# andreicuceu/vega

Measured on AMD Instinct MI355X. Metric: model+chi2 evals/sec (Lya auto+cross), higher is better.
Workload: dtype f64

## Files before the change

vega_amd/csrc/vegamx.hip:

```cpp
#include "vmx_device.h"
#include "vmx_fit.h"
#include "vmx_ensemble.h"
#include "vmx_nested.h"
#include "vmx_smc.h"
#include "vmx_chain.h"

#include <atomic>
#include <cmath>
#include <chrono>
#include <thread>
#include <algorithm>
#include <cstdio>
#include <cstdlib>
#include <cstring>
#include <map>
#include <mutex>
#include <queue>
#include <utility>
#include <string>
#include <vector>

#ifndef VMX_MAX_LANES
#define VMX_MAX_LANES 2
#endif
// ... 11 lines not shown
            return fail(-2, std::string(#call) + ": " + hipGetErrorString(err__));           \
    } while (0)

#define REQUIRE(cond, msg)                                                                   \
    do { if (!(cond)) return fail(-1, std::string("invalid argument: ") + msg); } while (0)

namespace {

static const uint64_t VMX_PART_SENTINEL = 0x7ff8dead0000beefull;


enum KernelClass {
    KC_PROLOGUE = 0, KC_PK, KC_FFTLOG, KC_XI, KC_METAL, KC_ASSEMBLE, KC_DISTORTION, KC_POST,
    KC_INVCOV, KC_CHI2, KC_MATVEC, KC_OTHER, KC_QUAD
};
const char* kKernelNames[VMX_N_KERNELS] = {
    "prologue", "pk_multipoles", "fftlog_spline_product", "xi_bins", "metal_matrix_product",
    "assemble", "distortion_product", "post", "invcov_product", "chi2", "matvec_api", "other",
    "quadratic_form_product"};

template <typename T>
struct DevBuf {
    T* p = nullptr;
    size_t n = 0;
    bool borrowed = false;
    DevBuf() = default;
    DevBuf(const DevBuf& o) : p(o.p), n(o.n), borrowed(true) {}
    DevBuf& operator=(const DevBuf& o) { if (this != &o) { release(); p = o.p; n = o.n; borrowed = true; } return *this; }
    void forget() { if (borrowed) { p = nullptr; n = 0; borrowed = false; } }
    int alloc(size_t count, bool zero = true) {
        release();
        if (count == 0) count = 1;
        hipError_t err = hipMalloc((void**)&p, count * sizeof(T));
        if (err != hipSuccess) return fail(-2, std::string("hipMalloc: ") + hipGetErrorString(err));
        n = count;
        if (zero) {
            err = hipMemset(p, 0, count * sizeof(T));
            if (err != hipSuccess) return fail(-2, std::string("hipMemset: ") + hipGetErrorString(err));
        }
        return 0;
    }
    int upload(const T* host, size_t count) {
        if (alloc(count, false)) return -2;
        hipError_t err = hipMemcpy(p, host, count * sizeof(T), hipMemcpyHostToDevice);
        if (err != hipSuccess) return fail(-2, std::string("hipMemcpy: ") + hipGetErrorString(err));
        return 0;
    }
    void release() { if (p && !borrowed) (void)hipFree(p); p = nullptr; n = 0; borrowed = false; }
    ~DevBuf() { release(); }
};

static int upload_padded(DevBuf<double>& buf, const double* host, int rows, int cols, int ld)
{
    if (buf.alloc((size_t)rows * ld, true)) return -2;
    hipError_t err = hipMemcpy2D(buf.p, (size_t)ld * sizeof(double), host, (size_t)cols * sizeof(double),
                                 (size_t)cols * sizeof(double), rows, hipMemcpyHostToDevice);
    if (err != hipSuccess) return fail(-2, std::string("hipMemcpy2D: ") + hipGetErrorString(err));
    return 0;
}

static std::vector<double> half_form(const double* c, int n)
{
    std::vector<double> out((size_t)n * n, 0.0);
    for (int i = 0; i < n; ++i) {
        for (int j = 0; j < i; ++j) out[(size_t)i * n + j] = 0.5 * (c[(size_t)i * n + j] + c[(size_t)j * n + i]);
        out[(size_t)i * n + i] = 0.5 * c[(size_t)i * n + i];
    }
    return out;
}

struct MetalHost {
    MetalDev dev{};
    DevBuf<double> mat, svec, basis, kron_a, kron_b;
    int rows = 0, cols = 0;
};

struct ItemHost {
    ItemDev dev{};
    std::vector<MetalHost*> metals;
    DevBuf<double> dm, cinv, data, vec, dist, res, z, mock_pool, add_vec;
    DevBuf<double> marg, marg_out;
    DevBuf<double> q_mat, q_w, q_lin, q_c0, q_x0, q_x, q_z;
    DevBuf<double> q_u, q_f, q_u0, q_y;
    DevBuf<double> mg_g, mg_c0, mg_y;
    DevBuf<double> mc_chol, mc_fid, q_cfull, q_m0, mc_z, mc_noise, mc_r0, mc_t;
    bool has_factor = false;
    std::vector<double> h_q_c0;
    DevBuf<int64_t> q_basis_off;
    int q_rows = 0;
    int n_templates = 0;
    int n_mocks = 0;
    DevBuf<int32_t> inv_mask;
    DevBuf<int64_t> csr_ptr; DevBuf<int32_t> csr_idx; DevBuf<double> csr_val;
    int64_t csr_nnz = 0; bool has_csr = false;
    std::vector<int32_t> mask_idx;
    bool has_dm = false, has_cinv = false, has_mask = false, has_data = false;
    bool lean_pair = false;
};

struct FitWorkspace {
    DevBuf<double> state;
    DevBuf<vmx_migrad::Spec> spec;
    DevBuf<double> base, theta, chi2;
    DevBuf<int32_t> mock_row, count, offset, done, mock, status;
    DevBuf<double> ox[vmx_migrad::MAX_STAGES], oext[vmx_migrad::MAX_STAGES], oV[vmx_migrad::MAX_STAGES], ofval[vmx_migrad::MAX_STAGES], oedm[vmx_migrad::MAX_STAGES];
    DevBuf<int32_t> oflags[vmx_migrad::MAX_STAGES], oiter[vmx_migrad::MAX_STAGES];
    DevBuf<int64_t> onfcn[vmx_migrad::MAX_STAGES];
    int32_t* pin_word = nullptr; int32_t* dpin_word = nullptr;
    std::vector<hipEvent_t> ev_gap;
    ~FitWorkspace() {
        if (pin_word) (void)hipHostFree(pin_word);
        for (auto& ev : ev_gap) (void)hipEventDestroy(ev);
    }
};
template <typename T>
static int ensure(DevBuf<T>& b, size_t count) { return b.n >= count && b.p ? 0 : b.alloc(count, false); }

struct BoxDev {
    double* theta; const double* chi2; const int32_t* status;
    const double* fixed; const int32_t* inv; const double* lo; const double* hi;
};
struct BoxWorkspace {
    DevBuf<double> theta, chi2, fixed, lo, hi;
    DevBuf<int32_t> status, inv;
    int upload(size_t rows, int P, int n, const double* h_fixed, const double* h_lo, const double* h_hi, const std::vector<int32_t>& h_inv,
               hipStream_t st, BoxDev& D)
    {
        if (ensure(theta, rows * P) || ensure(chi2, rows) || ensure(status, rows) || ensure(fixed, P) || ensure(inv, P) || ensure(lo, n) ||
            ensure(hi, n)) return -2;
        HIP_OK(hipMemcpyAsync(fixed.p, h_fixed, (size_t)P * sizeof(double), hipMemcpyHostToDevice, st));
        HIP_OK(hipMemcpyAsync(inv.p, h_inv.data(), (size_t)P * sizeof(int32_t), hipMemcpyHostToDevice, st));
        HIP_OK(hipMemcpyAsync(lo.p, h_lo, (size_t)n * sizeof(double), hipMemcpyHostToDevice, st));
        HIP_OK(hipMemcpyAsync(hi.p, h_hi, (size_t)n * sizeof(double), hipMemcpyHostToDevice, st));
        D = BoxDev{theta.p, chi2.p, status.p, fixed.p, inv.p, lo.p, hi.p};
        return 0;
    }
};

template <int THREADS, typename U>
__device__ inline void write_cube_rows(const BoxDev& B, int P, size_t row0, int rows, U u)
{
    for (int p = threadIdx.x % 64; p < P; p += 64) {
        const int d = B.inv[p];
        const double fixed = B.fixed[p], lo = d < 0 ? 0.0 : B.lo[d], hi = d < 0 ? 0.0 : B.hi[d];
#pragma unroll 4
        for (int r = threadIdx.x / 64; r < rows; r += THREADS / 64) {
            double v = fixed;
            if (d >= 0) v = vmx_ns::map_cube(lo, hi, u(r, d));
            B.theta[(row0 + (size_t)r) * P + p] = v;
        }
    }
}
template <int THREADS, typename U>
__device__ inline void write_cube_rows(const BoxDev& B, int P, int rows, U u)
{
    write_cube_rows<THREADS>(B, P, (size_t)0, rows, u);
}

struct EnsWorkspace {
    BoxWorkspace box;
    DevBuf<double> x, lnl, prop, factor, chain, chain_lnl;
    DevBuf<int64_t> acc, n_box, n_fail;
    DevBuf<int32_t> inside, col;
    DevBuf<int32_t> mock;
    DevBuf<uint64_t> streams;
    DevBuf<double> beta;
// ... 1349 lines not shown
}

struct SmcSetDev {
    SmcDev run0;
    const int32_t* active;
    const uint64_t* streams;
    const int64_t* stage0;
    const int32_t* mock_row;
    int32_t* mock;
    int32_t rec_rows;
};

__device__ __forceinline__ SmcDev smc_view(const SmcSetDev& S, int& run)
{
    SmcDev D = S.run0;
    const size_t a = blockIdx.x, r = (size_t)S.active[a], N = (size_t)D.N, n = (size_t)D.n;
    run = (int)r;
    D.u += r * N * n; D.lnl += r * N; D.u2 += r * N * n; D.lnl2 += r * N; D.w += r * N; D.cum += r * N;
    D.mean += r * n; D.cov += r * n * n; D.chol += r * n * n; D.state += r * 2;
    D.prop += r * N * n; D.uacc += r * N; D.inside += r * N;
    D.box.theta += a * N * (size_t)D.P; D.box.chi2 += a * N; D.box.status += a * N;
    D.rec += r * (size_t)S.rec_rows * VMX_SMC_REC; D.rec_lnl += r * (size_t)S.rec_rows * N; D.rec_anc += r * (size_t)S.rec_rows * N;
    D.counters += r * 3; D.host += r * 4;
    D.stream = S.streams[r];
    return D;
}

__device__ __forceinline__ void smc_write_mock(const SmcSetDev& S, int run)
{
    if (!S.mock_row) return;
    const int N = S.run0.N, m = S.mock_row[run];
    for (int i = threadIdx.x; i < N; i += SMC_THREADS) S.mock[(size_t)blockIdx.x * N + i] = m;
}

__global__ __launch_bounds__(SMC_THREADS) void k_smc_start(SmcSetDev S)
{
    int run;
    const SmcDev D = smc_view(S, run);
    smc_write_mock(S, run);
    smc_start(D);
}

__global__ __launch_bounds__(SMC_THREADS) void k_smc_start_lnl(SmcSetDev S)
{
    int run;
    const SmcDev D = smc_view(S, run);
    smc_start_lnl(D);
}

__global__ __launch_bounds__(SMC_THREADS) void k_smc_stage(SmcSetDev S, int64_t round)
{
    int run;
    const SmcDev D = smc_view(S, run);
    smc_stage(D, S.stage0[run] + round, round);
}

__global__ __launch_bounds__(SMC_THREADS) void k_smc_stage_kept(SmcSetDev S, int64_t round, double* rec_u)
{
    int run;
    const SmcDev D = smc_view(S, run);
    if (rec_u) rec_u += (size_t)run * (size_t)S.rec_rows * (size_t)D.N * (size_t)D.n;
    smc_stage<true>(D, S.stage0[run] + round, round, rec_u);
}

__global__ __launch_bounds__(SMC_THREADS) void k_smc_move(SmcSetDev S, int64_t round, int s_dec, int s_prop)
{
    int run;
    const SmcDev D = smc_view(S, run);
    if (s_dec < 0) smc_write_mock(S, run);
    smc_move(D, S.stage0[run] + round, s_dec, s_prop, round);
}

}

struct vmx_chain_store {
    vmx_engine* engine = nullptr;
    int E = 0, W = 0, n = 0;
    int64_t capacity = 0, rows = 0;
    DevBuf<double> x, lnl;
    DevBuf<double> sums, centred, out;
    DevBuf<int64_t> window;
};

struct vmx_engine {
    int device = 0;
    hipStream_t stream = nullptr;
    hipStream_t cur = nullptr;
    std::vector<hipStream_t> aux;
    hipEvent_t ev_fork = nullptr;
    std::vector<hipEvent_t> ev_join;
    bool finalized = false;
    std::vector<vmx_engine*> lanes;
    int n_lanes = 1;
    int64_t lane_calls = 0;
    hipStream_t last_stream = nullptr;
    const int32_t* call_mock = nullptr;
    FitWorkspace* fitws = nullptr;
    EnsWorkspace* ensws = nullptr;
    std::vector<vmx_chain_store*> chain_stores;
    vmx_chain_store* chain_store = nullptr;
    NsWorkspace* nsws = nullptr;
    SmcWorkspace* smcws = nullptr;
    hipEvent_t lane_wait = nullptr, ev_rows = nullptr, ev_lane = nullptr;

    int nk = 0, nkp = 0, n_mu = 0;
    int n_rows = 0, n_extra = 0, mu_lo = 0, mu_hi = 0;
    int mu_tiers = 1;
    vmx_plan::MuTierDesc mu_tier[vmx_plan::MU_TIERS] = {};
    std::vector<uint16_t> zmap64, zmap16;
    int last_tab2_kt = 0;
    DevBuf<double> node_w, mu_img, mu_img_w;
    std::vector<int32_t> rule_slot; std::vector<double> rule_lo, rule_hi;
    DevBuf<int32_t> d_rule_slot; DevBuf<double> d_rule_lo, d_rule_hi;
    double k_node_max = 0.0; bool mu_nodes_on = true;
    DevBuf<double> k, pklin, delta2, mu, sq1mmu2, lnmu, wl, gk, gk_mom, fv_x, fv_f, xtab;
    std::vector<int32_t> const_slots;
    std::vector<int32_t> const_slots2;
    DevBuf<int32_t> d_const_slots, d_const_slots2, d_xtab_pipe, d_xtab_partner;
    DevBuf<double> xtab_k;
    std::vector<int32_t> xi_static_taps, xi_static_bins;
    DevBuf<int32_t> d_xi_static_taps, d_xi_static_bins;
    DevBuf<unsigned long long> gemm_trace;
    size_t gemm_trace_blocks = 0;
    DevBuf<unsigned long long> pk_trace;
    size_t pk_trace_blocks = 0;
    std::vector<int32_t> w_groups;
    DevBuf<int32_t> d_w_groups;
    bool no_pk_w = false;
    std::vector<Tab2Group> tab2_groups;
    DevBuf<double> xtab_key;
    int n_xtab = 0;
    int const_hint = 0;
    int fv_n = 0;
    struct GkSpec { double rp, rt, mock_rp, mock_rt; };
    std::vector<GkSpec> gk_tables;
    std::vector<double> h_k, h_mu;

    int n_coef = 0, ncp = 0, n_knots = 0;
    DevBuf<double> op;
    bool op_set[VMX_MAX_ELL] = {false, false, false, false};
    bool extrapolate = false;
    double x0[VMX_MAX_ELL] = {0}, h[VMX_MAX_ELL] = {0};

    std::vector<PipeDev> pipes;
    std::vector<double> h_r, h_mu_c, h_z, h_relz, h_lnrelz, h_lnrelz2, h_growth;
    DevBuf<double> cr, cmu, crp, crt, cz, crelz, clnrelz, clnrelz2, cgrowth;
    DevBuf<PipeDev> d_pipes;
    std::vector<PkGroup> pk_groups;
    DevBuf<PkGroup> d_pk_groups;
    std::vector<int32_t> pk_members, pk_poly, pk_static;
    DevBuf<int32_t> d_pk_members, d_pk_poly, d_pk_static, d_pipe_active;
    DevBuf<double> poly_coef, poly_bins;
    int64_t poly_bins_total = 0;
    int n_active = 0;
    bool poly_dirty = true;

    std::vector<ItemHost*> items;
    std::vector<MetalHost*> metals;
    DevBuf<ItemDev> d_items;
    DevBuf<MetalDev> d_metals;
    std::vector<double> h_bb, h_odd, h_odd_op;
    std::map<int, int64_t> odd_op_off;
    DevBuf<double> bb_basis, odd_coef, odd_op, odd_dyn, sn_a;
    int sn_n = 0; double sn_tau0 = 0.0, sn_dtau = 1.0;

    std::vector<int32_t> prior_slot;
    std::vector<double> prior_mean, prior_sigma;
    DevBuf<int32_t> d_prior_slot;
    DevBuf<double> d_prior_mean, d_prior_sigma;

    DevBuf<double> gcinv, gres, gz;
    int g_n = 0, g_ld = 0;

    int n_params = 0, max_batch = 0, model_size = 0, slab_rows = 0;
    int pad_l = 0, pad_r = 0;
    int fact_slab_rows = 0;
    std::map<int, std::vector<int>> group_splits;
    struct QuadList { DevBuf<GemmWork> work; DevBuf<int32_t> queue, nt_off; DevBuf<double> part; int n_blocks = 0; int n_entries = 0; };
    std::map<int, QuadList*> quad_lists;
    std::vector<void*> host_allocs;
    std::map<int, QuadList*> cinv_lists;
    DevBuf<double> zero_row;
    int quad_blocks = 0;
    std::vector<double> host_key, pending_key;
    bool host_key_valid = false, skip_xtab_once = false;
    bool fft_ring = true, fft_ring_attr = false;
    bool xi_sums = true;
    bool sums_dirty = true;
    std::vector<XiLeanGroup> lean_groups; std::vector<XiStaticGroup> static_groups;
    std::vector<int32_t> lean_single;
    std::vector<int32_t> static_single;
    DevBuf<XiLeanGroup> d_lean_groups; DevBuf<XiStaticGroup> d_static_groups; DevBuf<ItemSums> d_item_sums;
    DevBuf<int32_t> d_static_single;
    bool sums_any = false;
    bool xi_lean = true;
    std::vector<int32_t> xi_lean_pipes, xi_rest_pipes;
    DevBuf<int32_t> d_xi_rest_pipes;
    bool ring_allowed = true;
    int last_tab_level = 0;
    bool no_tab2 = false;
    bool no_cinv_tape = false;
    bool pk_small_attr = false;
    bool kron_attr = false;
    DevBuf<double> mv_part;
    int64_t xi_total = 0, xim_total = 0;
    DevBuf<double> theta, scal, metal_bias, pl, coef, xi, xim, model, chi2;
    DevBuf<int32_t> status, mock_index, k_live, coef_win;
    DevBuf<double> pk_direct;
    bool direct = false;
    std::vector<int32_t> h_mock_index;
    int last_B = 0;
    bool last_full = false;
    bool last_taps = true;
    std::vector<double> theta_ref;
    bool quad_eligible = false, quad_mat_dirty = true, quad_lin_dirty = true, no_fuse = false;
    bool static_poly = true;
    int quad_kind = 0;
    bool quad_factored = false;
    struct MargReq { double* out; int64_t ld_out; int32_t* status; };
    const MargReq* marg_req = nullptr;
    int marg_slab_rows = 0;
    int last_form = 0;
    int last_route = 0, route_setup = 0;
    int last_fft_form = 0;
    struct ChainFacts { int route = 0; bool taps = true; int fft_form = 0; int tab2_kt = 0; };
    std::map<int, ChainFacts> graph_route;
    bool trace_host = false; double host_ns[3] = {0, 0, 0}; int64_t host_calls = 0;
    EngineDev dev{};

    double* pin_theta = nullptr; double* pin_chi2 = nullptr; int32_t* pin_status = nullptr;
    std::vector<double> blind_scale, blind_shift;
    DevBuf<double> d_blind;
    double* dpin_theta = nullptr; double* dpin_chi2 = nullptr; int32_t* dpin_status = nullptr;
    int64_t* pin_done = nullptr; int64_t* dpin_done = nullptr; int64_t done_seq = 0;
    double* pin_part = nullptr; double* dpin_part = nullptr;
    int host_reduce_items = 0, host_reduce_blocks[VMX_MAX_GROUP] = {0};
    bool no_host_reduce = false;
    std::map<int, hipGraphExec_t> graphs;
    bool use_graphs = true;

    bool profiling = false;
    uint32_t prof_mask = 0xffffffffu;
    int prof_stride = 1; int64_t prof_count[32] = {};
    struct Span { hipEvent_t a, b; int kc; };
    std::vector<Span> spans;
    size_t span_used = 0;
    double ms[VMX_N_KERNELS] = {0};
    int64_t launches[VMX_N_KERNELS] = {0};

    ~vmx_engine() {
        for (auto* l : lanes) { (void)hipStreamSynchronize(l->stream); delete l; }
        lanes.clear();
        for (auto* it : items) delete it;
        for (auto* m : metals) delete m;
        for (auto& s : spans) { (void)hipEventDestroy(s.a); (void)hipEventDestroy(s.b); }
        for (auto& g : graphs) (void)hipGraphExecDestroy(g.second);
        for (auto& q : quad_lists) delete q.second;
        for (auto& q : cinv_lists) delete q.second;
        for (void* p : host_allocs) (void)hipHostFree(p);
        delete fitws;
        delete ensws;
        for (auto* c : chain_stores) delete c;
        delete nsws;
        delete smcws;
        if (pin_theta) (void)hipHostFree(pin_theta);
        if (pin_chi2) (void)hipHostFree(pin_chi2);
        if (pin_status) (void)hipHostFree(pin_status);
        if (pin_done) (void)hipHostFree(pin_done);
        if (pin_part) (void)hipHostFree(pin_part);
        for (auto& a : aux) (void)hipStreamDestroy(a);
        for (auto& ev : ev_join) (void)hipEventDestroy(ev);
        if (ev_fork) (void)hipEventDestroy(ev_fork);
        if (ev_rows) (void)hipEventDestroy(ev_rows);
        if (ev_lane) (void)hipEventDestroy(ev_lane);
        if (stream) (void)hipStreamDestroy(stream);
    }
};

namespace {

static void drop_lane(vmx_engine* e)
{
    if (!e) return;
    for (auto* l : e->lanes) { (void)hipStreamSynchronize(l->stream); delete l; }
    e->lanes.clear();
}
static void wait_lane(vmx_engine* e) { if (e) for (auto* l : e->lanes) (void)hipStreamSynchronize(l->stream); }

struct ScopedTimer {
    vmx_engine* e; int idx = -1;
    ScopedTimer(vmx_engine* eng, int kc) : e(eng) {
        if (!e->profiling || !((e->prof_mask >> kc) & 1u)) return;
        if (e->prof_stride > 1 && (e->prof_count[kc]++ % e->prof_stride) != 0) return;
        if (e->span_used == e->spans.size()) {
            vmx_engine::Span s{};
            if (hipEventCreate(&s.a) != hipSuccess || hipEventCreate(&s.b) != hipSuccess) return;
            e->spans.push_back(s);
        }
        idx = (int)e->span_used++;
        e->spans[idx].kc = kc;
        (void)hipEventRecord(e->spans[idx].a, e->cur);
// ... 876 lines not shown
    return 0;
}

int vmx_host_free(vmx_engine* e, void* p)
{
    REQUIRE(e && p, "vmx_host_free");
    auto it = std::find(e->host_allocs.begin(), e->host_allocs.end(), p);
    REQUIRE(it != e->host_allocs.end(), "vmx_host_free: not a buffer of vmx_host_alloc on this engine");
    HIP_OK(hipSetDevice(e->device));
    HIP_OK(hipStreamSynchronize(e->stream));
    wait_lane(e);
    e->host_allocs.erase(it);
    HIP_OK(hipHostFree(p));
    return 0;
}

int vmx_set_mock_index(vmx_engine* e, const int32_t* index, int32_t B)
{
    REQUIRE(e && e->finalized, "vmx_set_mock_index (after vmx_finalize)");
    drop_lane(e);
    REQUIRE(B >= 0 && B <= e->max_batch, "batch exceeds max_batch");
    HIP_OK(hipSetDevice(e->device));
    for (int b = 0; b < e->max_batch; ++b) e->h_mock_index[b] = -1;
    if (index) {
        for (int b = 0; b < B; ++b) {
            for (auto* it : e->items) REQUIRE(index[b] < 0 || index[b] < it->n_mocks, "mock index exceeds the pool");
            e->h_mock_index[b] = index[b];
        }
    }
    HIP_OK(hipStreamSynchronize(e->stream));
    HIP_OK(hipMemcpy(e->mock_index.p, e->h_mock_index.data(), (size_t)e->max_batch * sizeof(int32_t), hipMemcpyHostToDevice));
    return 0;
}

int vmx_set_global_invcov(vmx_engine* e, const double* invcov, int32_t n)
{
    REQUIRE(e && invcov && n > 0, "vmx_set_global_invcov");
    drop_lane(e);
    HIP_OK(hipSetDevice(e->device));
    const std::vector<double> half = half_form(invcov, n);
    if (e->finalized) {
        REQUIRE(e->g_n == n, "global inverse covariance size changed");
        HIP_OK(hipStreamSynchronize(e->stream));
        HIP_OK(hipMemcpy2D(e->gcinv.p, (size_t)e->g_ld * sizeof(double), half.data(), (size_t)n * sizeof(double),
                           (size_t)n * sizeof(double), n, hipMemcpyHostToDevice));
        return 0;
    }
    e->g_n = n; e->g_ld = vmx_pad(n);
    return upload_padded(e->gcinv, half.data(), n, n, e->g_ld);
}

int vmx_add_prior(vmx_engine* e, int32_t slot, double mean, double sigma)
{
    REQUIRE(e && !e->finalized && slot >= 0 && sigma != 0.0, "vmx_add_prior");
    e->prior_slot.push_back(slot); e->prior_mean.push_back(mean); e->prior_sigma.push_back(sigma);
    return 0;
}

static int poly_basis_build(vmx_engine* e);
static int xi_sum_plan(vmx_engine* e);

int vmx_finalize(vmx_engine* e, int32_t n_params, int32_t max_batch)
{
    REQUIRE(e && !e->finalized, "vmx_finalize");
    REQUIRE(n_params > 0 && max_batch > 0, "n_params / max_batch");
    REQUIRE(e->nk > 0 && !e->pipes.empty() && !e->items.empty(), "template, pipelines and items are required");
    REQUIRE(e->items.size() <= 16, "at most 16 correlation items");
    REQUIRE(e->pipes.size() * sizeof(PipeDev) <= 48 * 1024, "too many pipelines for the prologue's descriptor stage");
    for (int i = 0; i < VMX_MAX_ELL; ++i) REQUIRE(e->op_set[i], "all four FFTLog operators are required");
    HIP_OK(hipSetDevice(e->device));
    const int Bm = max_batch;
    e->n_params = n_params; e->max_batch = Bm;
    e->slab_rows = Bm > 1024 ? Bm : 1024;
    e->fact_slab_rows = std::max(1024, std::min(4 * Bm, 8192));
    if (getenv("VMX_NO_GRAPH")) e->use_graphs = false;
    if (getenv("VMX_TRACE_HOST")) e->trace_host = true;
    {
        int cus = 256;
        if (hipDeviceGetAttribute(&cus, hipDeviceAttributeMultiprocessorCount, e->device) != hipSuccess || cus <= 0) { (void)hipGetLastError(); cus = 256; }
        e->quad_blocks = 2 * cus;
    }
    if (getenv("VMX_NO_TAB2")) e->no_tab2 = true;
    if (getenv("VMX_NO_CINV_TAPE")) e->no_cinv_tape = true;
    if (getenv("VMX_NO_PK_W")) e->no_pk_w = true;
    if (getenv("VMX_NO_HOST_REDUCE")) e->no_host_reduce = true;
    if (getenv("VMX_NO_XI_LEAN")) e->xi_lean = false;
    if (getenv("VMX_NO_XI_SUMS")) e->xi_sums = false;

    auto slot_ok = [&](int s) { return s < n_params; };
    for (auto& p : e->pipes) {
        const vmx_pipe_desc& d = p.d;
        const int slots[] = {d.tracer[0].bias_slot, d.tracer[0].bias_eta_slot, d.tracer[0].beta_slot,
                             d.tracer[0].vd_sigma_slot, d.tracer[0].alpha_slot, d.tracer[1].bias_slot,
                             d.tracer[1].bias_eta_slot, d.tracer[1].beta_slot, d.tracer[1].vd_sigma_slot,
                             d.tracer[1].alpha_slot, d.growth_rate_slot, d.bias_gamma_slot, d.bias_prim_slot,
                             d.lambda_uv_slot, d.bias_gamma_e_slot, d.lambda_heii_slot, d.bias_hcd_slot,
                             d.beta_hcd_slot, d.l0_hcd_slot, d.sigma_nl_par_slot, d.sigma_nl_per_slot,
                             d.exp_par_slot, d.exp_per_slot, d.scale_slot[0], d.scale_slot[1], d.drp_slot,
                             d.croom_slot[0], d.croom_slot[1], d.mock_los_slot};
        for (int s : slots) REQUIRE(slot_ok(s), "pipeline slot exceeds n_params");
        for (int i = 0; i < 6; ++i) REQUIRE(slot_ok(d.arinyo_slot[i]), "arinyo slot exceeds n_params");
        for (int i = 0; i < d.n_smooth; ++i)
            REQUIRE(d.smooth_par_slot[i] >= 0 && d.smooth_per_slot[i] >= 0 && slot_ok(d.smooth_par_slot[i]) &&
                    slot_ok(d.smooth_per_slot[i]), "smoothing slot");
        for (int q = 0; q < 2; ++q) {
            const vmx_tracer& t = d.tracer[q];
            const int have = (t.bias_slot >= 0) + (t.bias_eta_slot >= 0) + (t.beta_slot >= 0);
            REQUIRE(have >= 2, "each tracer needs two of (bias, bias_eta, beta)");
            REQUIRE(t.evol_kind == VMX_EVOL_CROOM ? (d.croom_slot[0] >= 0 && d.croom_slot[1] >= 0) : t.alpha_slot >= 0,
                    "bias-evolution slot");
            REQUIRE(d.vd_kind == VMX_VD_NONE || !t.discrete || t.vd_sigma_slot >= 0, "velocity dispersion slot");
        }
        REQUIRE(!d.uvb || (d.bias_gamma_slot >= 0 && d.bias_prim_slot >= 0 && d.lambda_uv_slot >= 0), "UVB slots");
        REQUIRE(!d.heii || (d.bias_gamma_e_slot >= 0 && d.bias_prim_slot >= 0 && d.lambda_heii_slot >= 0), "HeII slots");
        REQUIRE(d.hcd_model == VMX_HCD_NONE || (d.bias_hcd_slot >= 0 && d.beta_hcd_slot >= 0), "HCD slots");
        REQUIRE(d.hcd_model != VMX_HCD_ROGERS || d.l0_hcd_slot >= 0, "L0_hcd slot");
        REQUIRE(d.hcd_model != VMX_HCD_FVOIGT || e->fv_n >= 2, "model-hcd = fvoigt needs vmx_set_fvoigt_table");
        REQUIRE(d.nl_model != VMX_NL_ARINYO || (d.arinyo_slot[0] >= 0 && d.arinyo_slot[2] >= 0 && d.arinyo_slot[3] >= 0 &&
                                                d.arinyo_slot[4] >= 0 && d.arinyo_slot[5] >= 0), "Arinyo slots");
        REQUIRE(!d.peak_nl || d.sigma_nl_par_slot >= 0 || d.sigma_nl_per_slot >= 0, "sigmaNL slots");
        REQUIRE((d.exp_par_slot >= 0) == (d.exp_per_slot >= 0), "exp smoothing slots");
        REQUIRE(d.scale_mode == VMX_SCALE_UNIT || (d.scale_slot[0] >= 0 && d.scale_slot[1] >= 0), "scale slots");
        if (d.radiation) for (int i = 0; i < 4; ++i) REQUIRE(d.rad_slot[i] >= 0 && slot_ok(d.rad_slot[i]), "radiation slots");
        if (d.uv_shotnoise) {
            for (int i = 0; i < 3; ++i) REQUIRE(d.uvsn_slot[i] >= 0 && slot_ok(d.uvsn_slot[i]), "UV shot-noise slots");
            REQUIRE(e->sn_n >= 2, "UV shot noise needs vmx_set_shotnoise_table");
        }
    }
    for (auto* m : e->metals) {
        const vmx_metal_desc& d = m->dev.d;
        for (int q = 0; q < 2; ++q) {
            const vmx_tracer& t = d.tracer[q];
            REQUIRE(slot_ok(t.bias_slot) && slot_ok(t.bias_eta_slot) && slot_ok(t.beta_slot), "metal slot exceeds n_params");
            REQUIRE(!d.apply_bias || (t.bias_slot >= 0) + (t.bias_eta_slot >= 0) + (t.beta_slot >= 0) >= 2,
                    "each metal tracer needs two of (bias, bias_eta, beta)");
        }
        REQUIRE(slot_ok(d.growth_rate_slot) && slot_ok(d.extra_bias_slot), "metal slot exceeds n_params");
    }
    for (auto* it : e->items) {
        REQUIRE(slot_ok(it->dev.d.bao_amp_slot), "bao_amp slot exceeds n_params");
        REQUIRE(slot_ok(it->dev.add_slot), "additive-template slot exceeds n_params");
        for (int pos = 0; pos < 4; ++pos)
            for (int q = 0; q < it->dev.n_bb[pos]; ++q)
                for (int c = 0; c < it->dev.bb[pos][q].n_coef; ++c)
                    REQUIRE(slot_ok(it->dev.bb[pos][q].slot[c]), "broadband slot exceeds n_params");
    }

    const size_t gk_stride = (size_t)e->n_rows * e->nkp;
    if (!e->gk_tables.empty()) {
        if (e->gk.alloc(gk_stride * e->gk_tables.size() + (size_t)16 * e->nkp, true)) return -2;
        for (size_t t = 0; t < e->gk_tables.size(); ++t) {
            dim3 grid((e->nkp + 255) / 256, e->n_rows), block(256);
            hipLaunchKernelGGL(k_gk_table, grid, block, 0, e->stream, e->gk.p + t * gk_stride, e->k.p, e->mu.p,
                               e->nk, e->nkp, e->n_rows, e->gk_tables[t].rp, e->gk_tables[t].rt, e->gk_tables[t].mock_rp, e->gk_tables[t].mock_rt);
        }
        HIP_OK(hipGetLastError());
    }
    {
        const size_t nt = e->gk_tables.size();
        if (e->gk_mom.alloc((nt + 1) * 6 * (size_t)e->nkp, true)) return -2;
        for (size_t t = 0; t <= nt; ++t)
            hipLaunchKernelGGL(k_gk_moments, dim3((e->nkp + 63) / 64), dim3(64), 0, e->stream,
                               e->gk_mom.p + t * 6 * (size_t)e->nkp, t < nt ? e->gk.p + t * gk_stride : nullptr,
                               e->mu.p, e->nkp, e->n_mu);
        HIP_OK(hipGetLastError());
    }
// ... 259 lines not shown
    D.k = e->k.p; D.pklin = e->pklin.p; D.delta2 = e->delta2.p; D.mu = e->mu.p; D.sq1mmu2 = e->sq1mmu2.p; D.lnmu = e->lnmu.p;
    D.wl = e->wl.p; D.fv_x = e->fv_x.p; D.fv_f = e->fv_f.p; D.fv_n = e->fv_n; D.gk = e->gk.p; D.gk_mom = e->gk_mom.p; D.xtab = e->xtab.p; D.const_slots = e->d_const_slots.p; D.n_const_slots = 0; D.xtab_pipe = e->d_xtab_pipe.p; D.n_xtab = e->n_xtab; D.xtab_key = e->xtab_key.p; D.xtab_partner = e->d_xtab_partner.p; D.xtab_k = e->xtab_k.p; D.xtab_level = 0; D.n_gk = (int)e->gk_tables.size();
    D.n_coef = e->n_coef; D.ncp = e->ncp; D.extrapolate = e->extrapolate ? 1 : 0;
    for (int i = 0; i < VMX_MAX_ELL; ++i) {
        D.x0[i] = e->x0[i]; D.h[i] = e->h[i]; D.inv_h[i] = 1.0 / e->h[i]; D.xlast[i] = e->x0[i] + e->h[i] * (e->n_knots - 1);
    }
    D.same_grid = 1;
    for (int i = 1; i < VMX_MAX_ELL; ++i)
        if (e->op_set[i] && (!e->op_set[0] || D.x0[i] != D.x0[0] || D.inv_h[i] != D.inv_h[0] || D.xlast[i] != D.xlast[0])) D.same_grid = 0;
#ifdef VMX_EXP_NO_SAME_GRID
    D.same_grid = 0;
#endif
    D.n_pipe = n_pipe; D.pipes = e->d_pipes.p;
    D.n_active = e->n_active; D.n_static = (int)e->pk_static.size();
    if (!e->pk_static.empty() && e->poly_coef.alloc((size_t)VMX_MAX_ELL * e->pk_static.size() * 3 * e->ncp, true)) return -2;
    D.poly_coef = e->poly_coef.p;
    if (e->poly_bins_total > 0 && e->poly_bins.alloc((size_t)e->poly_bins_total, true)) return -2;
    D.poly_bins = e->poly_bins.p;
    D.cr = e->cr.p; D.cmu = e->cmu.p; D.crp = e->crp.p; D.crt = e->crt.p; D.cz = e->cz.p; D.crelz = e->crelz.p; D.clnrelz = e->clnrelz.p; D.clnrelz2 = e->clnrelz2.p; D.cgrowth = e->cgrowth.p;
    D.n_items = (int)e->items.size(); D.items = e->d_items.p;
    D.metals = e->d_metals.p; D.n_metals_total = (int)e->metals.size();
    D.bb_basis = e->bb_basis.p;
    D.odd_coef = e->odd_coef.p; D.odd_dyn = e->odd_dyn.p;
    D.sn_a = e->sn_a.p; D.sn_n = e->sn_n; D.sn_tau0 = e->sn_tau0; D.sn_dtau = e->sn_dtau;
    D.n_priors = (int)e->prior_slot.size();
    D.prior_slot = e->d_prior_slot.p; D.prior_mean = e->d_prior_mean.p; D.prior_sigma = e->d_prior_sigma.p;
    D.n_params = n_params;
    D.theta = e->theta.p; D.scal = e->scal.p; D.metal_bias = e->metal_bias.p; D.pl = e->pl.p; D.coef = e->coef.p;
    D.xi = e->xi.p; D.xim = e->xim.p; D.model = e->model.p; D.chi2 = e->chi2.p; D.status = e->status.p; D.k_live = e->k_live.p; D.coef_win = e->coef_win.p; D.pk_trace = nullptr; D.mock_index = e->mock_index.p;
    D.model_size = e->model_size;
    D.gcinv = e->gcinv.p; D.g_n = e->g_n; D.g_ld = e->g_ld; D.gres = e->gres.p; D.gz = e->gz.p;

    for (size_t q = 1; q < e->items.size(); ++q) {
        hipStream_t st = nullptr; hipEvent_t ev = nullptr;
        HIP_OK(hipStreamCreate(&st));
        HIP_OK(hipEventCreateWithFlags(&ev, hipEventDisableTiming));
        e->aux.push_back(st); e->ev_join.push_back(ev);
    }
    HIP_OK(hipEventCreateWithFlags(&e->ev_fork, hipEventDisableTiming));

    HIP_OK(hipHostMalloc((void**)&e->pin_theta, (size_t)Bm * n_params * sizeof(double), hipHostMallocMapped));
    HIP_OK(hipHostMalloc((void**)&e->pin_chi2, (size_t)Bm * sizeof(double), hipHostMallocMapped));
    HIP_OK(hipHostMalloc((void**)&e->pin_status, (size_t)Bm * sizeof(int32_t), hipHostMallocMapped));
    HIP_OK(hipHostMalloc((void**)&e->pin_done, sizeof(int64_t), hipHostMallocMapped));
    *e->pin_done = 0;
    if (hipHostMalloc((void**)&e->pin_part, (size_t)VMX_MAX_GROUP * 1024 * sizeof(double), hipHostMallocMapped) != hipSuccess ||
        hipHostGetDevicePointer((void**)&e->dpin_part, e->pin_part, 0) != hipSuccess) { (void)hipGetLastError(); e->dpin_part = nullptr; }
    if (getenv("VMX_NO_DONE_WORD") || hipHostGetDevicePointer((void**)&e->dpin_done, e->pin_done, 0) != hipSuccess) { (void)hipGetLastError(); e->dpin_done = nullptr; }
    if (!getenv("VMX_NO_ZERO_COPY") &&
        (hipHostGetDevicePointer((void**)&e->dpin_theta, e->pin_theta, 0) != hipSuccess ||
         hipHostGetDevicePointer((void**)&e->dpin_chi2, e->pin_chi2, 0) != hipSuccess ||
         hipHostGetDevicePointer((void**)&e->dpin_status, e->pin_status, 0) != hipSuccess)) {
        (void)hipGetLastError();
        e->dpin_theta = nullptr; e->dpin_chi2 = nullptr; e->dpin_status = nullptr;
    }

    e->quad_eligible = e->gcinv.p == nullptr && e->items.size() <= 16;
    for (auto* it : e->items) {
        int na = 0;
        if (it->dev.n_bb[VMX_BB_POST_MUL]) e->quad_eligible = false;
        for (int q = 0; q < it->dev.n_bb[VMX_BB_POST_ADD]; ++q) {
            if (it->dev.bb[VMX_BB_POST_ADD][q].func != VMX_BB_POLY) e->quad_eligible = false;
            na += it->dev.bb[VMX_BB_POST_ADD][q].n_coef;
        }
        if (na > VMX_MAX_QUAD_COEF) e->quad_eligible = false;
    }
    if (getenv("VMX_NO_QUAD")) e->quad_eligible = false;

    HIP_OK(hipStreamSynchronize(e->stream));
    e->finalized = true;
    if (poly_basis_build(e) || xi_sum_plan(e)) { e->finalized = false; return -2; }
    return 0;
}

int vmx_model_size(vmx_engine* e) { return e ? e->model_size : -1; }

int vmx_pipeline_column(vmx_engine* e, int32_t pipeline)
{
    REQUIRE(e && e->finalized && pipeline >= 0 && pipeline < (int)e->pipes.size(), "vmx_pipeline_column");
    return e->pipes[pipeline].col >= 0 ? e->pipes[pipeline].col : -3 - e->n_active;
}

constexpr double QUAD_ENTRY_STAGES = 4.0, QUAD_SKEW = 0.12;
constexpr bool QUAD_K_BANDS = true;

static vmx_engine::QuadList* quad_build_tape(vmx_engine* e, int B)
{
    const int tn = (B + GEMM_BN - 1) / GEMM_BN;
    std::vector<vmx_plan::TapeProblem> probs;
    for (auto* it : e->items) probs.push_back({it->dev.nq, it->dev.nq_pad});
    vmx_plan::Tape T = vmx_plan::plan_quad_tape(probs, tn, e->quad_blocks, QUAD_ENTRY_STAGES, QUAD_SKEW, GEMM_BM, GEMM_BK, QUAD_K_BANDS);
    auto* ql = new vmx_engine::QuadList();
    ql->n_blocks = T.n_blocks;
    ql->n_entries = (int)T.n_slots;
    if (T.work.empty()) T.work.push_back(GemmWork{-1, 0, 0, 0, 0, 0, 0, 0});
    if (ql->work.upload(T.work.data(), T.work.size()) || ql->queue.upload(T.queue.data(), T.queue.size()) ||
        ql->nt_off.upload(T.nt_off.data(), T.nt_off.size()) ||
        ql->part.alloc(std::max<size_t>((size_t)T.n_slots, 1) * 128, true)) { delete ql; return nullptr; }
    return ql;
}

static void quad_launch_list(vmx_engine* e, vmx_engine::QuadList* ql, int B)
{
    GemmGroup G{};
    for (size_t q = 0; q < e->items.size(); ++q) {
        ItemHost* it = e->items[q];
        const ItemDev& d = it->dev;
        GemmArgs g{};
        g.A = it->q_mat.p; g.lda = d.nq_pad; g.X = it->q_x.p; g.ldx = d.nq_pad; g.D = it->q_z.p; g.ldd = d.nq_pad;
        g.M = d.nq; g.N = B; g.K = d.nq_pad; g.tri = 1; g.nsplit = 1; g.klen = d.nq_pad;
        g.d_slab = (int64_t)B * d.nq_pad;
        g.tm = (d.nq + GEMM_BM - 1) / GEMM_BM; g.tn = (B + GEMM_BN - 1) / GEMM_BN;
        g.part = ql->part.p; g.lin = it->q_lin.p; g.lin_row = e->call_mock ? e->call_mock : e->mock_index.p; g.lin_pool = d.mock_pool ? 1 : 0;
        g.row0 = vmx_plan::tape_row0(d.nq, GEMM_BM);
        G.p[G.n++] = g;
    }
    G.work = ql->work.p;
    G.queue = ql->queue.p;
    if (getenv("VMX_QUAD_TRACE")) {
        e->gemm_trace_blocks = (size_t)ql->n_blocks;
        if (e->gemm_trace.n < 4 * e->gemm_trace_blocks) (void)e->gemm_trace.alloc(4 * e->gemm_trace_blocks, true);
        else (void)hipMemsetAsync(e->gemm_trace.p, 0, 4 * e->gemm_trace_blocks * sizeof(unsigned long long), e->cur);
        G.trace = e->gemm_trace.p;
    }
    hipLaunchKernelGGL((k_gemm_nt44<KC_QUAD>), dim3(ql->n_blocks, 1), dim3(GEMM44_THREADS), 0, e->cur, G);
}

static vmx_engine::QuadList* quad_work_list(vmx_engine* e, int B)
{
    const int tn = (B + GEMM_BN - 1) / GEMM_BN;
    auto found = e->quad_lists.find(tn);
    if (found != e->quad_lists.end()) return found->second;
    vmx_engine::QuadList* ql = quad_build_tape(e, B);
    if (ql) e->quad_lists[tn] = ql;
    return ql;
}

static bool cinv_tape_applies(const vmx_engine* e, int B)
{
    if (B <= 8 || e->no_cinv_tape) return false;
    if (e->gcinv.p) return true;
    if (e->items.size() > VMX_MAX_GROUP) return false;
    for (auto* it : e->items) if (!it->has_cinv) return false;
    return true;
}

static vmx_engine::QuadList* cinv_work_list(vmx_engine* e, int B)
{
    const int tn = (B + GEMM_BN - 1) / GEMM_BN;
    auto found = e->cinv_lists.find(tn);
    if (found != e->cinv_lists.end()) return found->second;
    std::vector<vmx_plan::TapeProblem> probs;
    int longest = 0;
    if (e->gcinv.p) { probs.push_back({e->g_n, e->g_ld}); longest = e->g_ld; }
    else for (auto* it : e->items) { probs.push_back({it->dev.n_masked, it->dev.n_masked_pad}); longest = std::max(longest, (int)it->dev.n_masked_pad); }
    if (e->zero_row.n < (size_t)longest && e->zero_row.alloc((size_t)longest, true)) return nullptr;
    vmx_plan::Tape T = vmx_plan::plan_quad_tape(probs, tn, e->quad_blocks, QUAD_ENTRY_STAGES, QUAD_SKEW, GEMM_BM, GEMM_BK, QUAD_K_BANDS);
    auto* ql = new vmx_engine::QuadList();
    ql->n_blocks = T.n_blocks;
    ql->n_entries = (int)T.n_slots;
    if (T.work.empty()) T.work.push_back(GemmWork{-1, 0, 0, 0, 0, 0, 0, 0});
    if (ql->work.upload(T.work.data(), T.work.size()) || ql->queue.upload(T.queue.data(), T.queue.size()) ||
        ql->nt_off.upload(T.nt_off.data(), T.nt_off.size()) ||
        ql->part.alloc(std::max<size_t>((size_t)T.n_slots, 1) * 128, true)) { delete ql; return nullptr; }
    e->cinv_lists[tn] = ql;
    return ql;
}

static void cinv_launch_list(vmx_engine* e, vmx_engine::QuadList* ql, int B)
{
    GemmGroup G{};
    auto add = [&](const double* A, const double* X, int n, int ld) {
        GemmArgs g{};
        g.A = A; g.lda = ld; g.X = X; g.ldx = ld; g.D = nullptr; g.ldd = ld;
        g.M = n; g.N = B; g.K = ld; g.tri = 1; g.nsplit = 1; g.klen = ld;
        g.d_slab = (int64_t)B * ld;
        g.tm = (n + GEMM_BM - 1) / GEMM_BM; g.tn = (B + GEMM_BN - 1) / GEMM_BN;
        g.part = ql->part.p; g.lin = e->zero_row.p; g.lin_row = nullptr; g.lin_pool = 0;
        g.row0 = vmx_plan::tape_row0(n, GEMM_BM);
        G.p[G.n++] = g;
    };
    if (e->gcinv.p) add(e->gcinv.p, e->gres.p, e->g_n, e->g_ld);
    else for (auto* it : e->items) add(it->cinv.p, it->res.p, it->dev.n_masked, it->dev.n_masked_pad);
    G.work = ql->work.p;
    G.queue = ql->queue.p;
    hipLaunchKernelGGL((k_gemm_nt44<KC_QUAD>), dim3(ql->n_blocks, 1), dim3(GEMM44_THREADS), 0, e->cur, G);
}

static int poly_basis_build(vmx_engine* e)
{
    e->poly_dirty = false;
    const int ns = (int)e->pk_static.size();
    e->xi_static_taps.clear(); e->xi_static_bins.clear();
    e->sums_dirty = true;
    if (ns == 0) return 0;
    DevBuf<double> V;
    const int64_t rows = (int64_t)ns * 3;
// ... 473 lines not shown
        launch_metal_kron(e, D, it, B);
        for (auto* m : it->metals) {
            if (m->dev.mat_off < 0 || m->dev.kron_a) continue;
            const PipeDev& P = e->pipes[m->dev.d.pipeline];
            launch_product(e, KC_METAL, m->mat.p, m->dev.mat_ld, 0, m->rows, m->dev.mat_ld,
                           e->xi.p + P.xi_off, P.n_pad, 0, B, e->xim.p + m->dev.xim_off, it->dev.n_model_pad, 0, 1, 0);
        }
    };
    if (quad) {
        e->cur = e->stream;
        int max_nq = 0;
        for (auto* it : e->items) { max_nq = std::max(max_nq, (int)it->dev.nq_pad); metal_products(it); }
        if (!xi_fused) {
            ScopedTimer t(e, KC_ASSEMBLE);
            hipLaunchKernelGGL(k_assemble_quad, dim3((max_nq + 255) / 256, B, (unsigned)e->items.size()), dim3(256), 0, e->cur, D);
        }
        if (e->marg_req) {
            e->last_form = e->quad_factored ? 2 : 1;
            if (marg_products(e, D, B, true)) return -2;
            e->last_B = B;
            e->last_full = false;
            return 0;
        }
        SlabInfo qs{};
        for (size_t q = 0; q < e->items.size(); ++q) qs.z[q] = 1;
        if (e->quad_factored) {
            if (B > 8 && e->items.size() <= VMX_MAX_GROUP) {
                GemmGroup G{};
                int tiles_total = 0, per_xcd_total = 0;
                for (auto* it : e->items) tiles_total += gemm_tiles(it->dev.n_masked, B, false);
                std::vector<size_t> by_size(e->items.size());
                for (size_t q = 0; q < by_size.size(); ++q) by_size[q] = q;
                std::stable_sort(by_size.begin(), by_size.end(), [&](size_t a, size_t b) {
                    const ItemDev& da = e->items[a]->dev; const ItemDev& db = e->items[b]->dev;
                    return (int64_t)da.n_masked * da.nq > (int64_t)db.n_masked * db.nq; });
                std::vector<int>& splits = e->group_splits[3 * 100000 + B];
                if (splits.empty()) {
                    std::vector<SplitProblem> sp;
                    for (size_t q : by_size) {
                        const ItemDev& d = e->items[q]->dev;
                        int max_split = 1;
                        while (max_split < 8 && (int64_t)max_split * 2 * B <= e->fact_slab_rows) max_split *= 2;
                        sp.push_back({gemm_tiles(d.n_masked, B, false), (d.nq_pad + GEMM_BK - 1) / GEMM_BK, (int64_t)B * d.n_masked_pad * 8, max_split,
                                      (d.n_masked + GEMM_BM - 1) / GEMM_BM, (B + GEMM_BN - 1) / GEMM_BN});
                    }
                    splits = choose_group_splits(sp, true);
                    if (splits.empty()) splits.push_back(0);
                }
                size_t gi = 0;
                for (size_t q : by_size) {
                    ItemHost* it = e->items[q];
                    const ItemDev& d = it->dev;
                    GemmArgs g{};
                    g.A = it->q_f.p; g.lda = d.nq_pad; g.X = it->q_x.p; g.ldx = d.nq_pad; g.D = it->q_y.p; g.ldd = d.n_masked_pad;
                    g.M = d.n_masked; g.N = B; g.K = d.nq_pad;
                    int per_xcd = 0;
                    const int forced = gi < splits.size() ? splits[gi] : 0;
                    ++gi;
                    qs.z[q] = plan_gemm(e, g, 1, e->fact_slab_rows, nullptr, false, tiles_total - gemm_tiles(d.n_masked, B, false), &per_xcd, forced);
                    per_xcd_total += per_xcd;
                    G.p[G.n] = g; G.seq_end[G.n] = per_xcd_total; ++G.n;
                }
                ScopedTimer t(e, KC_QUAD);
                launch_gemm_group(e, KC_QUAD, G, per_xcd_total, 1);
            } else {
                for (size_t q = 0; q < e->items.size(); ++q) {
                    ItemHost* it = e->items[q];
                    const ItemDev& d = it->dev;
                    qs.z[q] = launch_product(e, KC_QUAD, it->q_f.p, d.nq_pad, 0, d.n_masked, d.nq_pad, it->q_x.p, d.nq_pad, 0, B,
                                             it->q_y.p, d.n_masked_pad, 0, 1, e->fact_slab_rows);
                }
            }
            {
                ScopedTimer t(e, KC_CHI2);
                hipLaunchKernelGGL(k_chi2_quad<true>, dim3(B), dim3(CHI2_THREADS), 0, e->stream, D, B, qs);
            }
            HIP_OK(hipGetLastError());
            e->last_B = B;
            e->last_full = false;
            e->last_form = 2;
            return 0;
        }
        e->last_form = 1;
        if (B > 8 && e->items.size() <= VMX_MAX_GROUP) {
            vmx_engine::QuadList* ql = quad_work_list(e, B);
            if (!ql) return -2;
            {
                ScopedTimer t(e, KC_QUAD);
                quad_launch_list(e, ql, B);
            }
            ScopedTimer t(e, KC_CHI2);
#ifdef VMX_EXP_SKIP_SMALL
            static const int exp_skip1 = getenv("VMX_EXP_SKIP") ? atoi(getenv("VMX_EXP_SKIP")) : 0;
            static int exp_calls1 = 0;
            if (!((exp_skip1 & 1) && ++exp_calls1 > 64))
#endif
            hipLaunchKernelGGL(k_chi2_parts, dim3((B + 3) / 4), dim3(256), 0, e->stream, D, B, (const double*)ql->part.p,
                               (const int32_t*)ql->nt_off.p, 1);
            HIP_OK(hipGetLastError());
            e->last_B = B;
            e->last_full = false;
            return 0;
        } else if (B == 1 && D.done_host && e->dpin_part && !e->no_host_reduce && e->items.size() <= VMX_MAX_GROUP) {
            bool ok = true;
            for (auto* it : e->items) ok = ok && gemv1_applies(1, it->dev.nq_pad) && gemv1_blocks(it->dev.nq) <= 1024 && it->dev.nq_pad <= 2560 * 2;
            if (ok) {
                e->host_reduce_items = (int)e->items.size();
                for (size_t q = 0; q < e->items.size(); ++q) {
                    ItemHost* it = e->items[q];
                    const ItemDev& d = it->dev;
                    const int mock = (d.mock_pool && e->h_mock_index[0] >= 0) ? e->h_mock_index[0] : -1;
                    GemmArgs g{};
                    g.A = it->q_mat.p; g.lda = d.nq_pad; g.X = it->q_x.p; g.ldx = d.nq_pad; g.D = it->q_z.p; g.ldd = d.nq_pad;
                    g.M = d.nq; g.N = 1; g.K = d.nq_pad; g.tri = 1; g.nsplit = 1; g.klen = d.nq_pad;
                    g.part = e->dpin_part + q * 1024; g.lin = it->q_lin.p + (size_t)(mock >= 0 ? 1 + mock : 0) * d.nq_pad;
                    const int blocks = gemv1_blocks(d.nq);
                    e->host_reduce_blocks[q] = blocks;
                    ScopedTimer t(e, KC_QUAD);
                    const int last = q + 1 == e->items.size() ? 1 : 0;
                    if (d.nq_pad <= 2560) hipLaunchKernelGGL((k_gemv1<5, 2>), dim3(blocks), dim3(256), (size_t)d.nq_pad * sizeof(double), e->stream, g, D, last);
                    else hipLaunchKernelGGL((k_gemv1<10, 2>), dim3(blocks), dim3(256), (size_t)d.nq_pad * sizeof(double), e->stream, g, D, last);
                }
                HIP_OK(hipGetLastError());
                e->last_B = B;
                e->last_full = false;
                return 0;
            }
            for (size_t q = 0; q < e->items.size(); ++q) {
                ItemHost* it = e->items[q];
                const ItemDev& d = it->dev;
                qs.z[q] = launch_product(e, KC_QUAD, it->q_mat.p, d.nq_pad, 0, d.nq, d.nq_pad, it->q_x.p, d.nq_pad, 0, B,
                                         it->q_z.p, d.nq_pad, 0, 1, e->slab_rows, nullptr, -1, true);
            }
        } else {
            for (size_t q = 0; q < e->items.size(); ++q) {
                ItemHost* it = e->items[q];
                const ItemDev& d = it->dev;
                qs.z[q] = launch_product(e, KC_QUAD, it->q_mat.p, d.nq_pad, 0, d.nq, d.nq_pad, it->q_x.p, d.nq_pad, 0, B,
                                         it->q_z.p, d.nq_pad, 0, 1, e->slab_rows, nullptr, -1, true);
            }
        }
        {
            ScopedTimer t(e, KC_CHI2);
            hipLaunchKernelGGL(k_chi2_quad<false>, dim3(B), dim3(CHI2_THREADS), 0, e->stream, D, B, qs);
        }
        HIP_OK(hipGetLastError());
        e->last_B = B;
        e->last_full = false;
        return 0;
    }
    e->last_form = 0;
    SlabInfo slabs{};
    for (size_t q = 0; q < e->items.size(); ++q) slabs.z[q] = 1;
    const bool grouped = B > 8 && e->items.size() <= VMX_MAX_GROUP;
    if (grouped) {
        e->cur = e->stream;
        int max_model = 0, max_dist = 0;
        for (auto* it : e->items) {
            max_model = std::max(max_model, (int)it->dev.d.n_model); max_dist = std::max(max_dist, (int)it->dev.d.n_dist);
            metal_products(it);
        }
        {
            ScopedTimer t(e, KC_ASSEMBLE);
            hipLaunchKernelGGL(k_assemble_all, dim3((max_model + 255) / 256, B, (unsigned)e->items.size()), dim3(256), 0, e->cur, D);
        }
        SlabInfo dslabs{};
        for (size_t q = 0; q < e->items.size(); ++q) dslabs.z[q] = 1;
        for (int stage = 0; stage < 2; ++stage) {
            if (stage == 1 && (e->gcinv.p || cinv_tape_applies(e, B))) break;
            GemmGroup G{};
            int tiles_total = 0, per_xcd_total = 0;
            for (auto* it : e->items) {
// ... 168 lines not shown
        hipGraph_t graph = nullptr;
        HIP_OK(hipStreamBeginCapture(e->stream, hipStreamCaptureModeThreadLocal));
        const int rc = run_chain(e, B, tab_mode, zero_copy, nullptr, nullptr, nullptr, quad);
        hipError_t err = hipStreamEndCapture(e->stream, &graph);
        if (rc || err != hipSuccess || graph == nullptr) {
            if (graph) (void)hipGraphDestroy(graph);
            std::fprintf(stderr, "[vegamx] stream capture failed (%s): falling back to eager launches\n",
                         err != hipSuccess ? hipGetErrorString(err) : "launch error");
            (void)hipGetLastError();
            e->use_graphs = false;
            return run_chain(e, B, tab_mode, zero_copy, nullptr, nullptr, nullptr, quad);
        }
        hipGraphExec_t exec = nullptr;
        err = hipGraphInstantiate(&exec, graph, nullptr, nullptr, 0);
        (void)hipGraphDestroy(graph);
        if (err != hipSuccess) {
            std::fprintf(stderr, "[vegamx] graph instantiation failed (%s): falling back to eager launches\n", hipGetErrorString(err));
            e->use_graphs = false;
            return run_chain(e, B, tab_mode, zero_copy, nullptr, nullptr, nullptr, quad);
        }
        it = e->graphs.emplace(key, exec).first;
        vmx_engine::ChainFacts& captured = e->graph_route[key];
        captured.route = e->last_route;
        captured.taps = e->last_taps;
        captured.fft_form = e->last_fft_form;
        captured.tab2_kt = e->last_tab2_kt;
    }
    HIP_OK(hipGraphLaunch(it->second, e->stream));
    e->last_B = B;
    e->last_full = !quad;
    e->last_form = quad ? (e->quad_factored ? 2 : 1) : 0;
    const vmx_engine::ChainFacts& facts = e->graph_route[key];
    e->last_route = facts.route;
    e->last_taps = facts.taps;
    e->last_fft_form = facts.fft_form;
    e->last_tab_level = tab_mode;
    e->last_tab2_kt = facts.tab2_kt;
    return 0;
}

static int marg_fold_matrix(vmx_engine* e, ItemHost* it, const double* X)
{
    if (it->n_templates <= 0) return 0;
    const ItemDev& d = it->dev;
    if (it->mg_g.p == nullptr && it->mg_g.alloc((size_t)it->n_templates * d.nq_pad, true)) return -2;
    launch_product(e, KC_OTHER, X, d.n_masked_pad, 0, d.nq, d.n_masked_pad, it->marg.p, d.n_masked_pad, 0, it->n_templates,
                   it->mg_g.p, d.nq_pad, 0, 1, it->n_templates);
    return 0;
}

static int quad_build(vmx_engine* e)
{
    drop_lane(e);
    HIP_OK(hipStreamSynchronize(e->stream));
    const int P = e->n_params;
    std::vector<double> tref(e->theta_ref);
    if (!e->blind_scale.empty())
        for (int i = 0; i < P; ++i) tref[i] = e->blind_scale[i] == 1.0 ? tref[i] + e->blind_shift[i] : e->blind_scale[i] * tref[i] + e->blind_shift[i];
    HIP_OK(hipMemcpy(e->theta.p, tref.data(), (size_t)P * sizeof(double), hipMemcpyHostToDevice));
    e->no_fuse = true;
    const int rc = run_chain(e, 1, false);
    e->no_fuse = false;
    if (rc) return rc;
    HIP_OK(hipStreamSynchronize(e->stream));
    int32_t st = 0;
    HIP_OK(hipMemcpy(&st, e->status.p, sizeof(int32_t), hipMemcpyDeviceToHost));
    if (st) {
        std::fprintf(stderr, "[vegamx] the reference point of the quadratic chi2 form cannot be evaluated (status %d): full chain only\n", st);
        e->quad_eligible = false;
        return 0;
    }
    e->cur = e->stream;
    {
        double cost_q = 0.0, cost_f = 0.0;
        for (auto* it : e->items) {
            int na = 0;
            for (int q = 0; q < it->dev.n_bb[VMX_BB_POST_ADD]; ++q) na += it->dev.bb[VMX_BB_POST_ADD][q].n_coef;
            const double nq = it->dev.d.n_model + na;
            cost_q += nq * nq; cost_f += 2.0 * it->dev.n_masked * nq;
        }
        const bool fact = e->quad_kind == 2 || (e->quad_kind == 0 && cost_f < 0.75 * cost_q);
        if (fact != e->quad_factored) { e->quad_factored = fact; e->quad_mat_dirty = true; }
    }
    for (auto* it : e->items) {
        ItemDev& d = it->dev;
        const int nm = d.n_masked, nmp = d.n_masked_pad;
        int na = 0;
        std::vector<int64_t> boff;
        for (int q = 0; q < d.n_bb[VMX_BB_POST_ADD]; ++q) {
            const BBTermDev& term = d.bb[VMX_BB_POST_ADD][q];
            for (int c = 0; c < term.n_coef; ++c) { d.q_slot[na++] = term.slot[c]; boff.push_back(term.basis_off + (int64_t)c * d.d.n_dist); }
        }
        d.q_na = na; d.nq = d.d.n_model + na; d.nq_pad = vmx_pad(d.nq);
        {
            bool plain = d.d.pipe_peak != d.d.pipe_smooth;
            bool lean = plain;
            for (int pq : {d.d.pipe_peak, d.d.pipe_smooth}) {
                const PipeDev& P = e->pipes[pq];
                if (P.d.tracer[0].evol_kind != VMX_EVOL_STD || P.d.tracer[1].evol_kind != VMX_EVOL_STD ||
                    P.d.uv_shotnoise || P.odd_rel || P.odd_asy || P.poly_basis >= 0) { plain = false; lean = false; }
                if (P.d.radiation) plain = false;
            }
            const PipeDev& Pp = e->pipes[d.d.pipe_peak];
            const PipeDev& Ps = e->pipes[d.d.pipe_smooth];
            if (Pp.split_evol != Ps.split_evol || Pp.n != Ps.n) { plain = false; lean = false; }
            for (const std::vector<double>* h : {&e->h_r, &e->h_mu_c, &e->h_lnrelz, &e->h_lnrelz2, &e->h_growth})
                if ((plain || lean) && std::memcmp(h->data() + Pp.coord_off, h->data() + Ps.coord_off, (size_t)Pp.n * sizeof(double)) != 0) { plain = false; lean = false; }
            d.plain_pair = plain ? 1 : 0;
            it->lean_pair = lean;
        }
        const int nq = d.nq, nqp = d.nq_pad;
        REQUIRE(gemm44_addressable(nq, nqp) && gemm44_addressable(nq, nmp) && gemm44_addressable(nm, nqp),
                "quadratic form: " GEMM44_LIMIT_MSG);
        std::vector<double> x0((size_t)nqp, 0.0);
        HIP_OK(hipMemcpy(x0.data(), it->vec.p, (size_t)d.d.n_model * sizeof(double), hipMemcpyDeviceToHost));
        for (int j = 0; j < na; ++j) x0[d.d.n_model + j] = (e->direct ? 1.0 : 1.0 + tref[d.d.bao_amp_slot]) * tref[d.q_slot[j]];
        if (it->q_x0.upload(x0.data(), x0.size())) return -2;

        DevBuf<int32_t> midx;
        if (midx.upload(it->mask_idx.data(), it->mask_idx.size())) return -2;
        DevBuf<double>& cfull = it->q_cfull;
        if (it->has_cinv) {
            if (cfull.n < (size_t)nm * nmp && cfull.alloc((size_t)nm * nmp, true)) return -2;
            hipLaunchKernelGGL(k_sym_from_half, dim3((nm + 255) / 256, nm), dim3(256), 0, e->stream, cfull.p, it->cinv.p, nm, nmp);
        }
        if (it->q_m0.n < (size_t)nmp && it->q_m0.alloc((size_t)nmp, true)) return -2;
        hipLaunchKernelGGL(k_mask_gather, dim3((nm + 255) / 256), dim3(256), 0, e->stream, it->q_m0.p, (const double*)(e->model.p + d.model_off), midx.p, nm);
        if (e->quad_factored && (e->quad_mat_dirty || it->q_f.p == nullptr)) {
            std::vector<double> hu((size_t)nm * nmp, 0.0);
            if (it->has_cinv) {
                std::vector<double> hc((size_t)nm * nmp);
                HIP_OK(hipStreamSynchronize(e->stream));
                HIP_OK(hipMemcpy(hc.data(), cfull.p, hc.size() * sizeof(double), hipMemcpyDeviceToHost));
                if (!vmx_plan::cholesky_lower(hc.data(), nm, nmp)) {
                    std::fprintf(stderr, "[vegamx] the inverse covariance of an item is not positive definite: chi2 keeps the Q' form\n");
                    e->quad_kind = 1;
                    return quad_build(e);
                }
                for (int i = 0; i < nm; ++i)
                    for (int m = 0; m <= i; ++m) hu[(size_t)m * nmp + i] = hc[(size_t)i * nmp + m];
            } else
                for (int i = 0; i < nm; ++i) hu[(size_t)i * nmp + i] = 1.0;
            if (it->q_u.p == nullptr && it->q_u.alloc((size_t)nm * nmp, true)) return -2;
            HIP_OK(hipMemcpy(it->q_u.p, hu.data(), hu.size() * sizeof(double), hipMemcpyHostToDevice));
            DevBuf<double> X;
            DevBuf<int64_t>& bo = it->q_basis_off;
            boff.push_back(0);
            if (bo.upload(boff.data(), boff.size())) return -2;
            if (X.alloc((size_t)nq * nmp, true)) return -2;
            hipLaunchKernelGGL(k_quad_gather, dim3((nm + 255) / 256, nq), dim3(256), 0, e->stream, X.p, nmp,
                               it->has_dm ? it->dm.p : (const double*)nullptr, d.n_model_pad, midx.p, nm, (int)d.d.n_model, nq,
                               e->bb_basis.p, bo.p, (int)d.d.n_dist, it->has_csr ? 1 : 0);
            if (it->has_csr)
                hipLaunchKernelGGL(k_quad_gather_csr, dim3(nm), dim3(256), 0, e->stream, X.p, nmp, it->csr_ptr.p, it->csr_idx.p,
                                   it->csr_val.p, midx.p, nm);
            if (it->q_f.p == nullptr && it->q_f.alloc((size_t)nm * nqp, true)) return -2;
            launch_product(e, KC_OTHER, X.p, nmp, 0, nq, nmp, it->q_u.p, nmp, 0, nm, it->q_f.p, nqp, 0, 1, nm);
            if (marg_fold_matrix(e, it, X.p)) return -2;
            HIP_OK(hipStreamSynchronize(e->stream));
        }
        if (!e->quad_factored && (e->quad_mat_dirty || it->q_mat.p == nullptr)) {
            DevBuf<double> X, qfull;
            DevBuf<int64_t>& bo = it->q_basis_off;
            boff.push_back(0);
            if (bo.upload(boff.data(), boff.size())) return -2;
            if (X.alloc((size_t)nq * nmp, true)) return -2;
            hipLaunchKernelGGL(k_quad_gather, dim3((nm + 255) / 256, nq), dim3(256), 0, e->stream, X.p, nmp,
                               it->has_dm ? it->dm.p : (const double*)nullptr, d.n_model_pad, midx.p, nm, (int)d.d.n_model, nq,
                               e->bb_basis.p, bo.p, (int)d.d.n_dist, it->has_csr ? 1 : 0);
            if (it->has_csr)
                hipLaunchKernelGGL(k_quad_gather_csr, dim3(nm), dim3(256), 0, e->stream, X.p, nmp, it->csr_ptr.p, it->csr_idx.p,
                                   it->csr_val.p, midx.p, nm);
            if (it->q_w.p == nullptr && it->q_w.alloc((size_t)nq * nmp, true)) return -2;
            if (it->has_cinv)
                launch_product(e, KC_OTHER, cfull.p, nmp, 0, nm, nmp, X.p, nmp, 0, nq, it->q_w.p, nmp, 0, 1, nq);
            else
                HIP_OK(hipMemcpyAsync(it->q_w.p, X.p, (size_t)nq * nmp * sizeof(double), hipMemcpyDeviceToDevice, e->stream));
            if (qfull.alloc((size_t)nq * nqp, true)) return -2;
            launch_product(e, KC_OTHER, X.p, nmp, 0, nq, nmp, it->q_w.p, nmp, 0, nq, qfull.p, nqp, 0, 1, nq);
            if (it->q_mat.p == nullptr && it->q_mat.alloc((size_t)nq * nqp, true)) return -2;
            hipLaunchKernelGGL(k_half_from_full, dim3((nqp + 255) / 256, nq), dim3(256), 0, e->stream, it->q_mat.p, qfull.p, nq, nqp);
            if (marg_fold_matrix(e, it, X.p)) return -2;
            HIP_OK(hipStreamSynchronize(e->stream));
        }
        const int rows = 1 + it->n_mocks;
        DevBuf<double> R0, T;
        if (R0.alloc((size_t)rows * nmp, true)) return -2;
        hipLaunchKernelGGL(k_quad_rows, dim3((nm + 255) / 256, rows), dim3(256), 0, e->stream, R0.p, nmp,
                           (const double*)(e->model.p + d.model_off), midx.p, it->data.p,
                           it->n_mocks ? it->mock_pool.p : (const double*)nullptr, nm, rows);
        if (it->q_lin.alloc((size_t)rows * nqp, true) || it->q_c0.alloc(rows, true)) return -2;
        if (e->quad_factored) {
            if (it->q_u0.alloc((size_t)rows * nmp, true)) return -2;
            launch_product(e, KC_OTHER, it->q_u.p, nmp, 0, nm, nmp, R0.p, nmp, 0, rows, it->q_u0.p, nmp, 0, 1, rows);
            if (it->q_y.n < (size_t)e->fact_slab_rows * nmp && it->q_y.alloc((size_t)e->fact_slab_rows * nmp, true)) return -2;
            d.q_u0 = it->q_u0.p; d.q_y = it->q_y.p;
        } else
        launch_product(e, KC_OTHER, it->q_w.p, nmp, 0, nq, nmp, R0.p, nmp, 0, rows, it->q_lin.p, nqp, 0, 1, rows);
        if (e->quad_factored) {}
        else if (it->has_cinv) {
            if (T.alloc((size_t)rows * nmp, true)) return -2;
            launch_product(e, KC_OTHER, cfull.p, nmp, 0, nm, nmp, R0.p, nmp, 0, rows, T.p, nmp, 0, 1, rows);
            hipLaunchKernelGGL(k_rowdot, dim3(rows), dim3(256), 0, e->stream, it->q_c0.p, R0.p, T.p, nmp, nm);
        } else {
            hipLaunchKernelGGL(k_rowdot, dim3(rows), dim3(256), 0, e->stream, it->q_c0.p, R0.p, R0.p, nmp, nm);
        }
        if (it->n_templates > 0) {
            const int ldt = vmx_pad(it->n_templates);
            if (it->mg_c0.n != (size_t)rows * ldt && it->mg_c0.alloc((size_t)rows * ldt, true)) return -2;
            launch_product(e, KC_OTHER, it->marg.p, nmp, 0, it->n_templates, nmp, R0.p, nmp, 0, rows, it->mg_c0.p, ldt, 0, 1, rows);
        }
        it->q_rows = rows;
        if (it->q_x.n < (size_t)e->max_batch * nqp && it->q_x.alloc((size_t)e->max_batch * nqp, true)) return -2;
        if (!e->quad_factored && it->q_z.n < (size_t)e->slab_rows * nqp && it->q_z.alloc((size_t)e->slab_rows * nqp, true)) return -2;
        HIP_OK(hipGetLastError());
        HIP_OK(hipStreamSynchronize(e->stream));
        it->h_q_c0.resize(rows);
        HIP_OK(hipMemcpy(it->h_q_c0.data(), it->q_c0.p, (size_t)rows * sizeof(double), hipMemcpyDeviceToHost));
        d.q_x0 = it->q_x0.p; d.q_lin = it->q_lin.p; d.q_c0 = it->q_c0.p; d.q_x = it->q_x.p; d.q_z = it->q_z.p;
    }
    std::vector<ItemDev> items;
    for (auto* it : e->items) items.push_back(it->dev);
    HIP_OK(hipMemcpy(e->d_items.p, items.data(), items.size() * sizeof(ItemDev), hipMemcpyHostToDevice));
    e->quad_mat_dirty = false;
    e->quad_lin_dirty = false;
    e->last_B = 0;
    for (auto& g : e->graphs) (void)hipGraphExecDestroy(g.second);
    e->graphs.clear(); e->graph_route.clear();
    return 0;
}

static int quad_ready(vmx_engine* e, bool* use, int B)
{
    *use = false;
    if (!e->quad_eligible || e->theta_ref.empty() || e->direct) return 0;
    if (e->quad_mat_dirty || e->quad_lin_dirty) {
        if (quad_build(e)) return -2;
        if (!e->quad_eligible) return 0;
    }
    if (B > 8 && e->items.size() <= VMX_MAX_GROUP && !quad_work_list(e, B)) return -2;
    *use = true;
    return 0;
}

static vmx_engine* clone_lane(vmx_engine* e)
{
    auto* L = new vmx_engine(*e);
    L->lanes.clear(); L->n_lanes = 1; L->lane_calls = 0;
    L->chain_stores.clear(); L->chain_store = nullptr;
    L->fitws = nullptr; L->ensws = nullptr; L->nsws = nullptr; L->smcws = nullptr; L->lane_wait = nullptr; L->ev_rows = nullptr; L->ev_lane = nullptr; L->call_mock = nullptr;
    L->stream = nullptr; L->cur = nullptr; L->aux.clear(); L->ev_join.clear(); L->ev_fork = nullptr;
    L->graphs.clear(); L->graph_route.clear(); L->quad_lists.clear(); L->cinv_lists.clear(); L->host_allocs.clear(); L->spans.clear(); L->span_used = 0; L->profiling = false;
    L->pin_theta = nullptr; L->pin_chi2 = nullptr; L->pin_status = nullptr; L->pin_done = nullptr; L->pin_part = nullptr;
    L->dpin_theta = nullptr; L->dpin_chi2 = nullptr; L->dpin_status = nullptr; L->dpin_done = nullptr; L->dpin_part = nullptr;
    L->host_key_valid = false; L->pending_key.clear();
    std::map<MetalHost*, MetalHost*> metal_map;
    L->metals.clear();
    for (auto* m : e->metals) { auto* c = new MetalHost(*m); metal_map[m] = c; L->metals.push_back(c); }
    L->items.clear();
    for (auto* it : e->items) {
        auto* c = new ItemHost(*it);
        for (auto*& m : c->metals) m = metal_map[m];
        L->items.push_back(c);
    }
    auto fail_out = [&]() -> vmx_engine* { delete L; return nullptr; };
    if (hipStreamCreate(&L->stream) != hipSuccess) return fail_out();
    L->cur = L->stream;
    for (size_t q = 1; q < L->items.size(); ++q) {
        hipStream_t st = nullptr; hipEvent_t ev = nullptr;
        if (hipStreamCreate(&st) != hipSuccess || hipEventCreateWithFlags(&ev, hipEventDisableTiming) != hipSuccess) return fail_out();
        L->aux.push_back(st); L->ev_join.push_back(ev);
    }
    if (hipEventCreateWithFlags(&L->ev_fork, hipEventDisableTiming) != hipSuccess) return fail_out();
    const int Bm = e->max_batch, n_pipe = (int)e->pipes.size();
    const size_t ncols = (size_t)Bm * n_pipe, acols = (size_t)Bm * std::max(e->n_active, 1);
    for (auto* b : {&L->theta, &L->scal, &L->metal_bias, &L->pl, &L->coef, &L->xi, &L->xim, &L->model, &L->chi2, &L->xtab, &L->xtab_k,
                    &L->xtab_key, &L->gres, &L->gz, &L->mv_part, &L->pk_direct}) b->forget();
    for (auto* b : {&L->status, &L->k_live, &L->coef_win}) b->forget();
    L->gemm_trace.forget(); L->pk_trace.forget(); L->d_items.forget();
    if (L->theta.alloc((size_t)Bm * e->n_params) || L->scal.alloc(ncols * VMX_NS) ||
        L->metal_bias.alloc((size_t)Bm * 3 * (e->metals.size() + 1)) ||
        L->pl.alloc((size_t)VMX_MAX_ELL * acols * e->nkp) || L->coef.alloc((size_t)VMX_MAX_ELL * acols * e->ncp) ||
        L->xi.alloc((size_t)e->xi_total) || L->xim.alloc((size_t)e->xim_total) ||
        L->model.alloc((size_t)Bm * e->model_size) || L->chi2.alloc(Bm) || L->status.alloc(Bm) || L->k_live.alloc(8)) return fail_out();
    {
        const int32_t empty_window[2] = {0x7fffffff, -1};
        if (L->coef_win.upload(empty_window, 2)) return fail_out();
    }
    if (e->n_xtab > 0) {
        std::vector<double> key((size_t)2 * e->n_xtab * VMX_XTAB_KEY + 1, std::nan(""));
        if (L->xtab.alloc(((size_t)e->n_xtab * 2 * e->n_rows + 128) * e->nkp, true) || L->xtab_k.alloc((size_t)e->n_xtab * 4 * e->nkp, true) ||
            L->xtab_key.upload(key.data(), key.size())) return fail_out();
    }
    if (e->gcinv.p && (L->gres.alloc((size_t)Bm * e->g_ld, true) || L->gz.alloc((size_t)e->slab_rows * e->g_ld, true))) return fail_out();
    std::vector<ItemDev> items;
    for (auto* it : L->items) {
        ItemDev& d = it->dev;
        for (auto* b : {&it->vec, &it->dist, &it->res, &it->z, &it->marg_out, &it->q_x, &it->q_z, &it->q_y}) {
            const size_t n = b->n;
            b->forget();
            if (n > 0 && b != &it->marg_out && b->alloc(n, true)) return fail_out();
        }
        d.vec = it->vec.p; d.dist = it->dist.p; d.res = it->res.p; d.z = it->z.p; d.q_x = it->q_x.p; d.q_z = it->q_z.p; d.q_y = it->q_y.p;
        items.push_back(d);
    }
    if (L->d_items.upload(items.data(), items.size())) return fail_out();
// ... 2353 lines not shown
                    int spin = 0;
                    while (slot[i] == VMX_PART_SENTINEL && attempt == 0) {
                        if ((++spin & 255) == 0 && std::chrono::steady_clock::now() > spin_until) break;
                    }
                    uint64_t bits = slot[i];
                    if (bits == VMX_PART_SENTINEL) { complete = false; break; }
                    double v; std::memcpy(&v, &bits, sizeof(double));
                    c += v;
                }
            }
            for (int spin = 0; complete && *st_word == -1 && attempt == 0;) {
                if ((++spin & 255) == 0 && std::chrono::steady_clock::now() > spin_until) break;
            }
            if (*st_word == -1) complete = false;
        }
        if (!complete) { e->host_reduce_items = 0; return fail(-2, "single-walker chain: the device left a result slot unwritten after the stream drained"); }
        for (int q = 0; q < e->host_reduce_items; ++q) {
            const ItemHost* it = e->items[q];
            const int mock = (it->dev.mock_pool && e->h_mock_index[0] >= 0) ? e->h_mock_index[0] : -1;
            c += it->h_q_c0[mock >= 0 ? 1 + mock : 0];
        }
        for (size_t q = 0; q < e->prior_slot.size(); ++q) {
            const double dlt = e->pin_theta[e->prior_slot[q]] - e->prior_mean[q];
            c += dlt * dlt / (e->prior_sigma[q] * e->prior_sigma[q]);
        }
        int32_t st = *st_word;
        if (!(c == c) || c > 1e300 || c < -1e300) st |= VMX_STATUS_NONFINITE;
        e->pin_status[0] = st;
        e->pin_chi2[0] = st ? 1e100 : c;
        e->host_reduce_items = 0;
        waited = true;
    }
    if (!waited && B == 1 && zero_copy && !model && e->dpin_done && !e->profiling && e->n_params <= VMX_THETA_ARG_MAX) {
        const int64_t want = e->done_seq;
        volatile int64_t* word = e->pin_done;
        for (int64_t spin = 0; spin < (int64_t)1 << 26 && !waited; ++spin) waited = *word == want;
    }
    if (!waited && vmx_sync(e)) return -2;
    if (chi2) std::memcpy(chi2, e->pin_chi2, (size_t)B * sizeof(double));
    if (status) std::memcpy(status, e->pin_status, (size_t)B * sizeof(int32_t));
    if (e->trace_host) {
        const auto t_end = std::chrono::steady_clock::now();
        e->host_ns[0] += std::chrono::duration<double, std::nano>(t_staged - t_begin).count();
        e->host_ns[1] += std::chrono::duration<double, std::nano>(t_enqueued - t_staged).count();
        e->host_ns[2] += std::chrono::duration<double, std::nano>(t_end - t_enqueued).count();
        ++e->host_calls;
    }
    return 0;
}

int64_t vmx_debug_read(vmx_engine* e, int32_t what, int32_t index, double* out, int64_t capacity)
{
    if (!e || !e->finalized || !out || e->last_B <= 0) { fail(-1, "invalid argument: vmx_debug_read"); return -1; }
    if (hipSetDevice(e->device) != hipSuccess || hipStreamSynchronize(e->stream) != hipSuccess) { fail(-2, "hip sync"); return -2; }
    wait_lane(e);
    const int B = e->last_B;
    const double* src = nullptr; int64_t count = 0;
    if (what == 0) { src = e->pl.p; count = (int64_t)VMX_MAX_ELL * B * e->n_active * e->nkp; }
    else if (what == 1) {
        if (index < 0 || index >= (int)e->pipes.size()) { fail(-1, "invalid argument: pipeline index"); return -1; }
        if (!e->last_taps) { fail(-1, "the last evaluation (chi2 only, more than 8 walkers, no metal terms) did not store the per-pipeline bins: ask for a model"); return -1; }
        src = e->xi.p + e->pipes[index].xi_off; count = (int64_t)B * e->pipes[index].n_pad;
    } else if (what == 2) { src = e->coef.p; count = (int64_t)VMX_MAX_ELL * B * e->n_active * e->ncp; }
    else if (what == 3) {
        if (index < 0 || index >= (int)e->metals.size() || e->metals[index]->dev.mat_off < 0) { fail(-1, "invalid argument: metal without matrix"); return -1; }
        int n_model_pad = 0;
        for (auto* it : e->items) for (auto* m : it->metals) if (m == e->metals[index]) n_model_pad = it->dev.n_model_pad;
        src = e->xim.p + e->metals[index]->dev.xim_off; count = (int64_t)B * n_model_pad;
    }
    else if (what == 4) {
        if (capacity < 3) { fail(-1, "invalid argument: capacity too small"); return -1; }
        int32_t live[8] = {0, 0, 0, 0, 0, 0, 0, 0};
        if (hipMemcpy(live, e->k_live.p, 8 * sizeof(int32_t), hipMemcpyDeviceToHost) != hipSuccess) { fail(-2, "hipMemcpy"); return -2; }
        const int kt = e->last_tab_level >= 2 ? e->last_tab2_kt : 0;
        const bool tiered = kt > 0 && !(kt == 64 ? e->zmap64 : e->zmap16).empty();
        out[0] = live[0]; out[1] = e->dev.k_node_max;
        out[2] = vmx_plan::mu_mean_nodes(e->h_k.data(), e->nk, kt, live[1], tiered ? e->mu_tiers : 1, e->mu_tier);
        if (capacity >= 4) out[3] = live[1];
        if (capacity >= 5) out[4] = e->last_tab_level;
        if (capacity >= 7) { out[5] = live[2]; out[6] = live[3]; }
        if (capacity >= 9) out[8] = e->last_form;
        if (capacity >= 10) out[9] = e->last_route | e->route_setup;
        if (capacity >= 11) out[10] = e->last_fft_form;
        if (capacity >= 8) { out[7] = live[4]; return capacity >= 11 ? 11 : capacity >= 10 ? 10 : capacity >= 9 ? 9 : 8; }
        return capacity >= 7 ? 7 : capacity >= 5 ? 5 : capacity >= 4 ? 4 : 3;
    }
    else if (what == 5) {
        if (index < 0 || index >= (int)e->items.size()) { fail(-1, "invalid argument: item index"); return -1; }
        const ItemHost* it = e->items[index];
        const bool fused = B == 1 && it->has_dm && gemv1_applies(1, it->dev.n_model_pad) && !e->no_fuse;
        if (!e->last_full || fused) { fail(-1, "the last evaluation (chi2 only, or a single walker's fused distortion product) did not store the pre-distortion vector"); return -1; }
        src = it->vec.p; count = (int64_t)B * it->dev.n_model_pad;
    }
    else if (what == 6) { src = e->scal.p; count = (int64_t)B * (int64_t)e->pipes.size() * VMX_NS; }
    else if (what == 7) {
        static_assert(VMX_DEBUG_NS == VMX_NS, "vegamx.h states the row length of the scalars");
#define VMX_SCALAR_INDEX(name) S_##name,
        const int idx[] = {VMX_NS, VMX_DEBUG_SCALARS(VMX_SCALAR_INDEX)};
#undef VMX_SCALAR_INDEX
        const int64_t n = sizeof(idx) / sizeof(idx[0]);
        if (capacity < n) { fail(-1, "invalid argument: capacity too small"); return -1; }
        for (int64_t i = 0; i < n; ++i) out[i] = idx[i];
        return n;
    }
    else if (what == 8) {
        if (index < 0 || index >= (int)e->pipes.size()) { fail(-1, "invalid argument: pipeline index"); return -1; }
        const PipeDev& P = e->pipes[index];
        const double* arr[8] = {e->cr.p, e->crp.p, e->crt.p, e->cz.p, e->crelz.p, e->clnrelz.p, e->clnrelz2.p, e->cgrowth.p};
        if ((int64_t)8 * P.n > capacity) { fail(-1, "invalid argument: capacity too small"); return -1; }
        for (int a = 0; a < 8; ++a)
            if (hipMemcpy(out + (size_t)a * P.n, arr[a] + P.coord_off, (size_t)P.n * sizeof(double), hipMemcpyDeviceToHost) != hipSuccess) { fail(-2, "hipMemcpy"); return -2; }
        return (int64_t)8 * P.n;
    }
    else if (what == 9) {
        if (index < 0 || index >= (int)e->pipes.size()) { fail(-1, "invalid argument: pipeline index"); return -1; }
        if (capacity < 30) { fail(-1, "invalid argument: capacity too small"); return -1; }
        const EngineDev& D = e->dev;
        const PipeDev& P = e->pipes[index];
        int64_t n = 0;
        out[n++] = D.n_coef; out[n++] = D.ncp; out[n++] = D.same_grid; out[n++] = D.extrapolate; out[n++] = e->n_active;
        for (int l = 0; l < VMX_MAX_ELL; ++l) { out[n++] = D.x0[l]; out[n++] = D.h[l]; out[n++] = D.inv_h[l]; out[n++] = D.xlast[l]; }
        out[n++] = P.col; out[n++] = P.n; out[n++] = P.n_pad; out[n++] = P.split_evol; out[n++] = P.poly_basis;
        out[n++] = P.poly_bins_off >= 0 ? 1 : 0; out[n++] = P.odd_x0; out[n++] = P.odd_h; out[n++] = P.odd_ncoef;
        return n;
    }
    else if (what == 10 || what == 11) {
        if (index < 0 || index >= (int)e->items.size()) { fail(-1, "invalid argument: item index"); return -1; }
        const ItemHost* it = e->items[index];
        if (e->last_full || e->last_form == 0 || !it->q_x.p || !it->q_x0.p) { fail(-1, "the last evaluation was not a chi2-only evaluation of the quadratic form: no x' - x0'"); return -1; }
        src = what == 10 ? it->q_x.p : it->q_x0.p; count = (what == 10 ? (int64_t)B : 1) * it->dev.nq_pad;
    }
    else if (what == 12) {
        if (index < 0 || index >= (int)e->pipes.size()) { fail(-1, "invalid argument: pipeline index"); return -1; }
        const PipeDev& P = e->pipes[index];
        if (P.poly_bins_off < 0 || !e->poly_bins.p) { fail(-1, "none: the pipeline has no static basis on its bins"); return -1; }
        src = e->poly_bins.p + P.poly_bins_off; count = (int64_t)3 * P.n_pad;
    }
    else if (what == 13 || what == 14 || what == 18 || what == 19) {
        const bool lean = what < 18, describe = what == 13 || what == 18;
        const int ng = (int)(lean ? e->lean_groups.size() : e->static_groups.size());
        if (describe && (index < 0 || index >= ng)) {
            if (capacity < 1) { fail(-1, "invalid argument: capacity too small"); return -1; }
            out[0] = ng;
            return 1;
        }
        if (index < 0 || index >= ng) { fail(-1, "invalid argument: group index"); return -1; }
        auto serve = [&](const auto& G) -> int64_t {
            if (describe) {
                if (capacity < 5 + 3 * G.n_members) { fail(-1, "invalid argument: capacity too small"); return -1; }
                int64_t n = 0;
                out[n++] = ng; out[n++] = G.n_members; out[n++] = G.n; out[n++] = G.n_pad; out[n++] = G.presum;
                for (int m = 0; m < G.n_members; ++m) { out[n++] = G.m[m].pipe; out[n++] = G.m[m].fkind; out[n++] = G.m[m].findex; }
                return n;
            }
            if (!(e->last_route & (lean ? VMX_ROUTE_GROUP : VMX_ROUTE_STATIC_GROUP))) { fail(-1, "the last evaluation did not sum its bins on the way: no group array"); return -1; }
            src = e->xi.p + G.out_off; count = (int64_t)B * G.n_pad;
            return 0;
        };
        const int64_t served = lean ? serve(e->lean_groups[index]) : serve(e->static_groups[index]);
        if (served != 0) return served;
    }
    else if (what == 15) { src = e->poly_coef.p; count = (int64_t)VMX_MAX_ELL * (int64_t)e->pk_static.size() * 3 * e->ncp; if (count == 0) { fail(-1, "none: no pipeline has a static coefficient basis"); return -1; } }
    else if (what == 16) {
        if (index < 0 || index >= (int)e->pipes.size()) { fail(-1, "invalid argument: pipeline index"); return -1; }
        const PipeDev& P = e->pipes[index];
        if (!P.odd_rel && !P.odd_asy) { fail(-1, "none: the pipeline has no odd-multipole terms"); return -1; }
        src = e->odd_coef.p + P.odd_off; count = (int64_t)4 * P.odd_ncoef;
    }
    else if (what == 17) { src = e->metal_bias.p; count = (int64_t)B * 3 * (int64_t)e->metals.size(); if (count == 0) { fail(-1, "none: no metal terms"); return -1; } }
    else { fail(-1, "invalid argument: what"); return -1; }
    if (count > capacity) { fail(-1, "invalid argument: capacity too small"); return -1; }
    if (hipMemcpy(out, src, (size_t)count * sizeof(double), hipMemcpyDeviceToHost) != hipSuccess) { fail(-2, "hipMemcpy"); return -2; }
    return count;
}

__global__ __launch_bounds__(256) void k_debug_math(int which, const double* x, double* out, int64_t n)
{
    const int64_t i = (int64_t)blockIdx.x * 256 + threadIdx.x;
    if (i >= n) return;
    const double v = x[i];
    out[i] = which == 0 ? vmx_log(v) : which == 1 ? vmx_exp(v) : vmx_rsqrt(v);
}

int vmx_debug_math(vmx_engine* e, int32_t which, const double* x, int64_t n, double* out)
{
    REQUIRE(e && x && out && n > 0 && n <= ((int64_t)1 << 30) && which >= 0 && which <= 2, "vmx_debug_math");
    wait_lane(e);
    HIP_OK(hipSetDevice(e->device));
    DevBuf<double> dx, dy;
    if (dx.upload(x, (size_t)n) || dy.alloc((size_t)n, false)) return -2;
    hipLaunchKernelGGL(k_debug_math, dim3((unsigned)((n + 255) / 256)), dim3(256), 0, e->stream, (int)which, dx.p, dy.p, n);
    HIP_OK(hipGetLastError());
    HIP_OK(hipStreamSynchronize(e->stream));
    HIP_OK(hipMemcpy(out, dy.p, (size_t)n * sizeof(double), hipMemcpyDeviceToHost));
    return 0;
}

int vmx_matvec_device(vmx_engine* e, const double* d_A, int32_t rows, int32_t cols, const double* d_x, int32_t B,
                      double* d_y)
{
    REQUIRE(e && d_A && d_x && d_y, "vmx_matvec_device");
    wait_lane(e);
    REQUIRE(rows > 0 && cols > 0 && cols % VMX_PAD == 0, "cols (leading dimension) must be a multiple of 32, zero padded");
    REQUIRE(B > 0, "vmx_matvec_device: B > 0");
    HIP_OK(hipSetDevice(e->device));
    const int ldy = vmx_pad(rows);
    REQUIRE(B <= 8 || (gemm44_addressable(rows, cols) && gemm44_addressable(B, cols)), "vmx_matvec_device with more than 8 vectors: " GEMM44_LIMIT_MSG);
    if (B <= 8) {
        launch_product(e, KC_MATVEC, d_A, cols, 0, rows, cols, d_x, cols, 0, B, d_y, ldy, 0, 1, 0);
    } else {
        const size_t need = (size_t)8 * B * ldy;
        if (e->mv_part.n < need) {
            HIP_OK(hipStreamSynchronize(e->stream));
            if (e->mv_part.alloc(need, false)) return -2;
        }
        const int ns = launch_product(e, KC_MATVEC, d_A, cols, 0, rows, cols, d_x, cols, 0, B, e->mv_part.p, ldy, 0, 1, 8 * B);
        const int64_t count = (int64_t)B * ldy;
        hipLaunchKernelGGL(k_sum_slabs, dim3((unsigned)((count + 255) / 256)), dim3(256), 0, e->cur, e->mv_part.p, d_y, count, ns);
    }
    HIP_OK(hipGetLastError());
    return 0;
}

int vmx_matmul_host(vmx_engine* e, const double* A, int32_t rows, int32_t cols, const double* X, int32_t B, double* Y)
{
    REQUIRE(e && A && X && Y && rows > 0 && cols > 0 && B > 0, "vmx_matmul_host");
    wait_lane(e);
    HIP_OK(hipSetDevice(e->device));
    HIP_OK(hipStreamSynchronize(e->stream));
    const int ld = vmx_pad(cols), ldy = vmx_pad(rows);
    DevBuf<double> dA, dX, dY;
    if (upload_padded(dA, A, rows, cols, ld) || upload_padded(dX, X, B, cols, ld) || dY.alloc((size_t)B * ldy, true)) return -2;
    if (vmx_matvec_device(e, dA.p, rows, ld, dX.p, B, dY.p)) return -2;
    HIP_OK(hipStreamSynchronize(e->stream));
    HIP_OK(hipMemcpy2D(Y, (size_t)rows * sizeof(double), dY.p, (size_t)ldy * sizeof(double), (size_t)rows * sizeof(double), B,
                       hipMemcpyDeviceToHost));
    return 0;
}

int vmx_set_profiling(vmx_engine* e, int32_t enabled)
{
    REQUIRE(e, "vmx_set_profiling");
    wait_lane(e);
    HIP_OK(hipSetDevice(e->device));
    HIP_OK(hipStreamSynchronize(e->stream));
    if (e->profiling) collect_spans(e);
    e->profiling = enabled != 0;
    e->prof_mask = 0xffffffffu;
    e->prof_stride = 1;
    while (e->profiling && e->spans.size() < 96) {
        vmx_engine::Span s{};
        HIP_OK(hipEventCreate(&s.a));
// ... 35 lines not shown
```

vega_amd/csrc/vmx_device.h:

```cpp
#pragma once
#include <hip/hip_runtime.h>
#include <stdint.h>
#include "../../include/vegamx.h"
#include "vmx_plan.h"

#define VMX_NS 40
#define VMX_PAD 32
#define VMX_MAX_BB 32
#define VMX_MAX_METALS 64
#define VMX_MAX_QUAD_COEF 64
#define VMX_MAX_GROUP 8
#define VMX_MAX_MARG 16

enum {
    S_BIAS1 = 0, S_BB1, S_BIAS2, S_BB2,
    S_UV_BG, S_UV_BP, S_UV_LAM, S_HE_BG, S_HE_LAM,
    S_HCD_B, S_HCD_BB, S_HCD_L0,
    S_GA, S_GB, S_EA, S_EB,
    S_AQ1, S_AQ2, S_AKV, S_AAV, S_ABV, S_AKP,
    S_VD1, S_VD2,
    S_AP, S_AT, S_DRP, S_EV1A, S_EV1B, S_EV2A, S_EV2B,
    S_RAD_S, S_RAD_A, S_RAD_L, S_RAD_D, S_RAD_IL, S_RAD_ID,
    S_NO_RULE
};
// ... 1945 lines not shown
            const double x = it.q_x[(size_t)b * it.nq_pad + i];
            double zs[8];
#pragma unroll
            for (int s = 0; s < 8; ++s) zs[s] = it.q_z[((size_t)(s < ns ? s : 0) * B + b) * it.nq_pad + i];
            double z = zs[0];
#pragma unroll
            for (int s = 1; s < 8; ++s) z += s < ns ? zs[s] : 0.0;
            acc = fma(x, 2.0 * (z - g[i]), acc);
        }
        if (threadIdx.x == 0) acc += it.q_c0[row];
    }
    for (int off = 32; off > 0; off >>= 1) acc += __shfl_down(acc, off, 64);
    if ((threadIdx.x & 63) == 0) red[threadIdx.x >> 6] = acc;
    __syncthreads();
    if (threadIdx.x == 0) {
        double c = 0.0;
        for (int w = 0; w < CHI2_THREADS / 64; ++w) c += red[w];
        const double* t = D.theta + (size_t)b * D.n_params;
        for (int q = 0; q < D.n_priors; ++q) {
            const double dlt = t[D.prior_slot[q]] - D.prior_mean[q];
            c += dlt * dlt / (D.prior_sigma[q] * D.prior_sigma[q]);
        }
        int st = D.status[b];
        if (!(c == c) || c > 1e300 || c < -1e300) { st |= VMX_STATUS_NONFINITE; D.status[b] = st; }
        D.chi2[b] = st ? 1e100 : c;
        if (D.chi2_host) D.chi2_host[b] = st ? 1e100 : c;
        if (D.status_host) D.status_host[b] = st;
        if (D.done_host) { __threadfence_system(); *D.done_host = D.done_seq; }
        if (b == 0) {
            D.k_live[2] = D.coef_win[0]; D.k_live[3] = D.coef_win[1]; D.coef_win[0] = 0x7fffffff; D.coef_win[1] = -1;
            xtab_key_store(D);
        }
    }
}

__global__ __launch_bounds__(256) void k_chi2_parts(EngineDev D, int B, const double* part, const int32_t* nt_off, int with_c0)
{
    const int b = blockIdx.x * 4 + (threadIdx.x >> 6), lane = threadIdx.x & 63;
    if (b >= B) return;
    const int nt = b >> 6, nl = b & 63;
    constexpr int CHI2_PRE = 4;
    const int s0 = nt_off[nt], s1 = nt_off[nt + 1];
    const int n_c0 = with_c0 ? D.n_items : 0;
    const int mock = with_c0 ? D.mock_index[b] : -1;
    int st = D.status[b];
    double c0[CHI2_PRE];
#pragma unroll
    for (int q = 0; q < CHI2_PRE; ++q) {
        c0[q] = 0.0;
        if (q < n_c0) { const ItemDev& it = D.items[q]; c0[q] = it.q_c0[(mock >= 0 && it.mock_pool) ? 1 + mock : 0]; }
    }
    double acc = 0.0;
    for (int j = s0 + lane; j < s1; j += 64) {
        const double* pp = part + ((size_t)j * 64 + nl) * 2;
        acc += pp[0] + pp[1];
    }
    for (int off = 32; off > 0; off >>= 1) acc += __shfl_down(acc, off, 64);
    if (lane != 0) return;
    double c = acc;
#pragma unroll
    for (int q = 0; q < CHI2_PRE; ++q) if (q < n_c0) c += c0[q];
    for (int q = CHI2_PRE; q < n_c0; ++q) {
        const ItemDev& it = D.items[q];
        c += it.q_c0[(mock >= 0 && it.mock_pool) ? 1 + mock : 0];
    }
    const double* t = D.theta + (size_t)b * D.n_params;
    for (int q = 0; q < D.n_priors; ++q) {
        const double dlt = t[D.prior_slot[q]] - D.prior_mean[q];
        c += dlt * dlt / (D.prior_sigma[q] * D.prior_sigma[q]);
    }
    if (!(c == c) || c > 1e300 || c < -1e300) { st |= VMX_STATUS_NONFINITE; D.status[b] = st; }
    D.chi2[b] = st ? 1e100 : c;
    if (D.chi2_host) D.chi2_host[b] = st ? 1e100 : c;
    if (D.status_host) D.status_host[b] = st;
#ifdef VMX_EXP_SKIP_SMALL
    if (b == 0) { D.k_live[2] = D.coef_win[0]; D.k_live[3] = D.coef_win[1]; xtab_key_store(D); return; }
#endif
    if (b == 0) {
        D.k_live[2] = D.coef_win[0]; D.k_live[3] = D.coef_win[1]; D.coef_win[0] = 0x7fffffff; D.coef_win[1] = -1;
        xtab_key_store(D);
    }
}

struct MargOutItem { const double* y; const double* c0; int32_t item, n, ld, off, slabs, pad; };
struct MargOutArgs { MargOutItem p[VMX_MAX_MARG]; double* out; int64_t ld_out; int32_t* status_out; int32_t finish; };

__global__ __launch_bounds__(256) void k_marg_out(EngineDev D, MargOutArgs A, int B)
{
    const int b = blockIdx.x;
    const MargOutItem& m = A.p[blockIdx.y];
    const ItemDev& it = D.items[m.item];
    const int st = D.status[b];
    const int mock = D.mock_index[b];
    const int row = (mock >= 0 && it.mock_pool) ? 1 + mock : 0;
    const double* c0 = m.c0 ? m.c0 + (size_t)row * m.ld : nullptr;
    double* out = A.out + (size_t)b * A.ld_out + m.off;
    for (int t = threadIdx.x; t < m.n; t += 256) {
        double y = 0.0;
        for (int s = 0; s < m.slabs; ++s) y += m.y[((size_t)s * B + b) * m.ld + t];
        const double v = c0 ? c0[t] - y : y;
        out[t] = st ? __longlong_as_double(0x7ff8000000000000ll) : v;
    }
    if (blockIdx.y == 0 && threadIdx.x == 0) {
        if (A.status_out) A.status_out[b] = st;
        if (A.finish && b == 0) {
            D.k_live[2] = D.coef_win[0]; D.k_live[3] = D.coef_win[1]; D.coef_win[0] = 0x7fffffff; D.coef_win[1] = -1;
            xtab_key_store(D);
        }
    }
}

__global__ void k_quad_gather(double* X, int ldx, const double* dm, int dm_ld, const int32_t* mask_idx, int n_masked,
                              int n_model, int nq, const double* bb_basis, const int64_t* basis_off, int n_dist, int csr)
{
    const int i = blockIdx.x * blockDim.x + threadIdx.x;
    const int j = blockIdx.y;
    if (i >= n_masked || j >= nq) return;
    const int r = mask_idx[i];
    double v;
    if (j < n_model) {
        if (csr) return;
        v = dm ? dm[(size_t)r * dm_ld + j] : (r == j ? 1.0 : 0.0);
    } else v = bb_basis[basis_off[j - n_model] + r];
    X[(size_t)j * ldx + i] = v;
}

__global__ void k_sym_from_half(double* full, const double* half, int n, int ld)
{
    const int j = blockIdx.x * blockDim.x + threadIdx.x, i = blockIdx.y;
    if (i >= n || j >= n) return;
    full[(size_t)i * ld + j] = i > j ? half[(size_t)i * ld + j] : i < j ? half[(size_t)j * ld + i] : 2.0 * half[(size_t)i * ld + i];
}

__global__ void k_half_from_full(double* half, const double* full, int n, int ld)
{
    const int j = blockIdx.x * blockDim.x + threadIdx.x, i = blockIdx.y;
    if (i >= n || j >= ld) return;
    double v = 0.0;
    if (j < i) v = 0.5 * (full[(size_t)i * ld + j] + full[(size_t)j * ld + i]);
    else if (j == i) v = 0.5 * full[(size_t)i * ld + i];
    half[(size_t)i * ld + j] = v;
}

__global__ void k_quad_rows(double* R0, int ld, const double* model0, const int32_t* mask_idx, const double* data,
                            const double* pool, int n_masked, int n_rows)
{
    const int i = blockIdx.x * blockDim.x + threadIdx.x, k = blockIdx.y;
    if (i >= n_masked || k >= n_rows) return;
    const double d = k == 0 ? data[i] : pool[(size_t)(k - 1) * n_masked + i];
    R0[(size_t)k * ld + i] = d - model0[mask_idx[i]];
}

__global__ void k_mask_gather(double* out, const double* model0, const int32_t* mask_idx, int n_masked)
{
    const int i = blockIdx.x * blockDim.x + threadIdx.x;
    if (i < n_masked) out[i] = model0[mask_idx[i]];
}

__global__ void k_mock_rows(double* pool, double* R0, int ld, const double* noise, const double* fid, const double* m0, int n_masked, int n_rows)
{
    const int i = blockIdx.x * blockDim.x + threadIdx.x, k = blockIdx.y;
    if (i >= n_masked || k >= n_rows) return;
    const double v = fid[i] + noise[(size_t)k * ld + i];
    pool[(size_t)k * n_masked + i] = v;
    if (R0) R0[(size_t)k * ld + i] = v - m0[i];
}
// ... 226 lines not shown
    v += dpp_move<0x124>(v);
    v += dpp_move<0x4e>(v);
    return v + dpp_move<0xb1>(v);
}
__device__ __forceinline__ double sum_k_quarters(double v)
{
    v += dpp_move<0x128>(v);
    return v + dpp_move<0x124>(v);
}

#ifndef GEMM44_THREADS
#define GEMM44_THREADS 256
#endif
template <int TAG, int NBUF = 2, int BNT = 64>
__global__ __launch_bounds__(GEMM44_THREADS, NBUF == 2 ? GEMM44_THREADS / 128 : 1) void k_gemm_nt44(GemmGroup G)
{
    constexpr int BM = 64, BN = BNT, BK = 32;
    constexpr int NT = GEMM44_THREADS, NW = NT / 64;
    static_assert(BN == 64 || (BN == 32 && NT == 256 && NBUF == 2), "the 32-walker tile exists for the four-wave, two-buffer kernel");
    constexpr int FJ = 4 * 256 / NT * 2;
    constexpr int NI = BN == 64 ? 8 : 4;
    constexpr int AR = BN == 64 ? 1 : 2;
    constexpr int NP = 16 / NW;
    constexpr int NPX = BN / 4 / NW;
    __shared__ double sA_static[NBUF == 2 ? 2 : 1][NBUF == 2 ? BM * BK : 1];
    __shared__ double sX_static[NBUF == 2 ? 2 : 1][NBUF == 2 ? BN * BK : 1];
    extern __shared__ double s_ring[];
    double (*sA)[BM * BK] = NBUF == 2 ? (double (*)[BM * BK])&sA_static[0][0] : (double (*)[BM * BK])s_ring;
    double (*sX)[BN * BK] = NBUF == 2 ? (double (*)[BN * BK])&sX_static[0][0] : (double (*)[BN * BK])(s_ring + NBUF * BM * BK);
    auto wait_stages = [](int ahead) {
        if (ahead >= 3) asm volatile("s_waitcnt vmcnt(%0)" ::"n"(3 * 2 * NP) : "memory");
        else if (ahead == 2) asm volatile("s_waitcnt vmcnt(%0)" ::"n"(2 * 2 * NP) : "memory");
        else if (ahead == 1) asm volatile("s_waitcnt vmcnt(%0)" ::"n"(1 * 2 * NP) : "memory");
        else asm volatile("s_waitcnt vmcnt(0)" ::: "memory");
    };
    constexpr bool QUAD = TAG == VMX_TAG_QUAD && NT == 256 && NBUF == 2 && BN == 64;
    __shared__ double sL[QUAD ? 2 * BM : 1];

    const bool persist = QUAD && G.work != nullptr && G.queue != nullptr;
    const bool list = persist;
    const unsigned long long t_start = G.trace ? wall_clock64() : 0ull;
    unsigned long long t_first = 0ull, t_loop = 0ull;
#ifdef VMX_EPI_TRACE
    unsigned long long t_e1 = 0ull, t_e2 = 0ull;
#endif
    GemmWork wk{};
    int bx = blockIdx.x, by = blockIdx.y;
    if constexpr (TAG == VMX_TAG_FFTLOG) {
        if (G.batch_in_x > 0) { const int s2 = bx >> 3; by = s2 % G.batch_in_x; bx = ((s2 / G.batch_in_x) << 3) | (bx & 7); }
    }
    int w_first = bx, w_count = 1;
    if (persist) { w_first = G.queue[blockIdx.x]; w_count = G.queue[blockIdx.x + 1] - w_first; if (w_count <= 0) return; }
    if (list) { wk = G.work[w_first]; if (wk.prob < 0) return; }
    const int xcd = bx & 7;
    int seq = bx >> 3;
    int pi = 0;
    if (list) pi = wk.prob;
    else {
        while (pi < G.n - 1 && seq >= G.seq_end[pi]) ++pi;
        if (pi > 0) seq -= G.seq_end[pi - 1];
    }
    const GemmArgs& g = G.p[pi];
    const int split = list ? wk.slab : xcd % g.nsplit, group = xcd / g.nsplit, ngroups = 8 / g.nsplit;
    const int tm_eff = g.tri ? (g.tm + 1) / 2 : g.tm;
    const bool n_major = !list && g.m_window != nullptr && g.nsplit == 1 && !g.tri;
    const int tnx = (g.tn + 7) / 8;
    int tm_live = tm_eff;
    if (n_major) {
        const int w_lo = max(g.m_window[0], 0), w_hi = min(g.m_window[1], g.M - 1);
        tm_live = w_hi >= w_lo ? (w_hi - w_lo) / BM + 1 : 0;
        if (tm_live == 0) return;
    }
    const int mt0 = list ? wk.mt : n_major ? seq % tm_live : (seq / g.tn) * ngroups + group;
    const int nt = list ? wk.nt : n_major ? (seq / tm_live) * 8 + xcd : seq % g.tn;
    if (!list && (mt0 >= tm_eff || nt >= g.tn)) return;
    const int npass = persist ? w_count : (!list && g.tri && g.tm - 1 - mt0 != mt0) ? 2 : 1;
    const int batch = by;
    const char* A = (const char*)(g.A + batch * g.a_batch);
    const char* X = (const char*)(g.X + batch * g.x_batch);
    double* Dp = g.D + batch * g.d_batch + split * g.d_slab;
    int p_M = g.M, p_N = g.N, p_lda = g.lda, p_ldx = g.ldx, p_lin_pool = g.lin_pool, p_row0 = g.row0;
    int p_mend = g.M;
    double* p_part = g.part;
    const double* p_lin = g.lin;
    const int32_t* p_lin_row = g.lin_row;

    const int tid = threadIdx.x, lane = tid & 63;
    const int wave = __builtin_amdgcn_readfirstlane(tid >> 6);
    const int wm = NT == 256 ? (wave & 1) * 32 : (wave & 3) * 16, wn = NT == 256 ? (wave >> 1) * (BN / 2) : (wave >> 2) * 32;
    const int fq = lane & 3, fb = (lane >> 2) & 3, fkk = lane >> 4;
    const unsigned frag0 = (unsigned)(((2 * fkk + (fb >> 1)) ^ (4 * fq)) * 16 + (fb & 1) * 8);
    const unsigned fa = lds_offset(&sA[0][(wm + fq) * BK]), fx = lds_offset(&sX[0][(wn + fq) * BK]);
    const int drow = lane >> 4;
    const unsigned dchunk = (unsigned)(((lane & 15) ^ (4 * drow)) * 16);
    int n0 = nt * BN;

    int m0 = 0, kbeg = 0, kend = 0;
    int slot = blockIdx.x;
    bool skip = false;
    unsigned oa[NP], ox[NPX];
    const int m_base = n_major ? max(g.m_window[0], 0) : 0;
    auto setup = [&](int pass) {
        if (persist) {
            wk = G.work[w_first + pass];
            const GemmArgs& q = G.p[__builtin_amdgcn_readfirstlane(wk.prob)];
            A = (const char*)q.A; X = (const char*)q.X;
            p_M = q.M; p_N = q.N; p_lda = q.lda; p_ldx = q.ldx; p_lin_pool = q.lin_pool; p_row0 = q.row0;
            p_part = q.part; p_lin = q.lin; p_lin_row = q.lin_row;
            n0 = wk.nt * BN;
            slot = wk.slot;
        }
        const int mt = persist ? wk.mt : pass == 0 ? mt0 : g.tm - 1 - mt0;
        m0 = m_base + mt * BM;
        p_mend = p_M;
        if (persist && p_row0 > 0) {
            m0 = mt == 0 ? 0 : p_row0 + (mt - 1) * BM;
            if (mt == 0) p_mend = p_row0;
        }
        if (list) { kbeg = wk.kbeg; kend = wk.kend; }
        else if (g.tri) {
            int kmax = ((mt + 1) * BM + BK - 1) / BK * BK; if (kmax > g.K) kmax = g.K;
            const int klen = ((kmax + g.nsplit - 1) / g.nsplit + BK - 1) / BK * BK;
            kbeg = split * klen; kend = kbeg + klen; if (kend > kmax) kend = kmax;
        } else {
            kbeg = split * g.klen; kend = kbeg + g.klen; if (kend > g.K) kend = g.K;
        }
        if (g.k_limit) { const int kl = (*g.k_limit + BK - 1) / BK * BK; if (kend > kl) kend = kl; }
        skip = g.m_window && (m0 + BM <= g.m_window[0] || m0 > g.m_window[1]);
#pragma unroll
        for (int p = 0; p < NP; ++p) {
            int r = m0 + (p * NW + wave) * 4 + drow; if (r >= p_M) r = p_M - 1;
            oa[p] = (unsigned)(r * p_lda) * 8u + dchunk;
        }
#pragma unroll
        for (int p = 0; p < NPX; ++p) {
            int r = n0 + (p * NW + wave) * 4 + drow; if (r >= p_N) r = p_N - 1;
            ox[p] = (unsigned)(r * p_ldx) * 8u + dchunk;
        }
    };
    auto dma_stage = [&](int k, int buf) {
#pragma unroll
        for (int p = 0; p < NP; ++p) {
            __builtin_amdgcn_global_load_lds((const __attribute__((address_space(1))) void*)(A + (oa[p] + (unsigned)k * 8u)),
                                             (__attribute__((address_space(3))) void*)&sA[buf][(p * NW + wave) * 4 * BK], 16, 0, 0);
            if (p < NPX)
                __builtin_amdgcn_global_load_lds((const __attribute__((address_space(1))) void*)(X + (ox[p] + (unsigned)k * 8u)),
                                                 (__attribute__((address_space(3))) void*)&sX[buf][(p * NW + wave) * 4 * BK], 16, 0, 0);
        }
    };
    setup(0);
    int first_buf = 0;
    if (!skip && kbeg < kend) dma_stage(kbeg, first_buf);

  for (int pass = 0; pass < npass; ++pass) {
    const int c_m0 = m0, kbeg_c = kbeg, kend_c = kend, c_n0 = n0, c_slot = slot, c_first = first_buf;
    const int c_M = p_mend, c_N = p_N, c_ldx = p_ldx, c_lin_pool = p_lin_pool;
    double* const c_part = p_part;
    const double* const c_lin = p_lin;
    const int32_t* const c_lin_row = p_lin_row;
    const bool c_skip = skip;

    double acc[NI][FJ];
#pragma unroll
    for (int i = 0; i < NI; ++i)
#pragma unroll
        for (int j = 0; j < FJ; ++j) acc[i][j] = 0.0;

    double a0[FJ], x0[NI], a1[FJ], x1[NI];
    if (!c_skip && kbeg_c < kend_c) {
        if constexpr (NBUF == 2) {
            asm volatile("s_waitcnt vmcnt(0)" ::: "memory");
            __syncthreads();
            if (kbeg_c + BK < kend_c) dma_stage(kbeg_c + BK, c_first ^ 1);
            if constexpr (QUAD) {
                if (list && c_part && wave == 0 && kbeg_c == 0 && !c_lin_pool) {
                    const unsigned loff = (unsigned)(c_m0 + 2 * lane < c_ldx ? (c_m0 + 2 * lane) * 8 : 0);
                    __builtin_amdgcn_global_load_lds((const __attribute__((address_space(1))) void*)((const char*)c_lin + loff),
                                                     (__attribute__((address_space(3))) void*)&sL[0], 16, 0, 0);
                }
            }
        } else {
            int ahead = 0;
#pragma unroll
            for (int q = 1; q < NBUF; ++q)
                if (kbeg_c + q * BK < kend_c) { dma_stage(kbeg_c + q * BK, q); ++ahead; }
            wait_stages(ahead);
            __syncthreads();
        }
        if (G.trace) t_first = wall_clock64();
        lds_read_fragments<4 * BK * 8>(a0, fa + (unsigned)c_first * (BM * BK * 8) + frag0);
        lds_read_fragments<4 * BK * 8>(x0, fx + (unsigned)c_first * (BN * BK * 8) + frag0);
        lds_wait(a0, x0);
    }
    int buf = NBUF == 2 ? c_first : 0;
    int epi_buf = -1;
    for (int k0 = kbeg_c; k0 < (c_skip ? kbeg_c : kend_c); k0 += BK) {
        const int nbuf = NBUF == 2 ? buf ^ 1 : (buf + 1 == NBUF ? 0 : buf + 1);
        const unsigned a1p = fa + (unsigned)buf * (BM * BK * 8) + (frag0 ^ 128u);
        const unsigned x1p = fx + (unsigned)buf * (BN * BK * 8) + (frag0 ^ 128u);
#define VMX_G44_FIRST(i)                                                                                              \
        if constexpr (i < NI) {                                                                                           \
            if constexpr (AR * i < FJ) a1[AR * i] = lds_read_b64<AR * i * 4 * BK * 8>(a1p);                               \
            if constexpr (AR == 2) a1[AR * i + 1] = lds_read_b64<(AR * i + 1) * 4 * BK * 8>(a1p);                        \
            x1[i] = lds_read_b64<i * 4 * BK * 8>(x1p);                                                                   \
            _Pragma("unroll") for (int j = 0; j < FJ; ++j)                                                               \
                acc[i][j] = __builtin_amdgcn_mfma_f64_4x4x4f64(x0[i], a0[j], acc[i][j], 0, 0, 0);                        \
            __builtin_amdgcn_sched_barrier(0);                        \
        }
        VMX_G44_FIRST(0) VMX_G44_FIRST(1) VMX_G44_FIRST(2) VMX_G44_FIRST(3)
        VMX_G44_FIRST(4) VMX_G44_FIRST(5) VMX_G44_FIRST(6) VMX_G44_FIRST(7)
#undef VMX_G44_FIRST
        lds_wait(a1, x1);
        if constexpr (NBUF == 2) asm volatile("s_waitcnt vmcnt(0)" ::: "memory");
        else {
            const int left = (kend_c - k0) / BK - 2;
            wait_stages(left < 0 ? 0 : left > NBUF - 2 ? NBUF - 2 : left);
        }
        __builtin_amdgcn_s_barrier();
        __builtin_amdgcn_sched_barrier(0);
        if (k0 + NBUF * BK < kend_c) dma_stage(k0 + NBUF * BK, buf);
        else if constexpr (QUAD) {
            if (epi_buf < 0 && list && c_part) {
                epi_buf = buf;
                const unsigned coff = (unsigned)(c_m0 + 2 * (lane & 31) < c_ldx ? (c_m0 + 2 * (lane & 31)) * 8 : 0);
#pragma unroll
                for (int p = 0; p < 8; ++p) {
                    const int pr = p * NW + wave;
                    int r = c_n0 + 2 * pr + (lane >> 5); if (r >= c_N) r = c_N - 1;
                    double* dst = pr < 16 ? &sA[buf][2 * pr * BM] : &sX[buf][(2 * pr - 32) * BM];
                    __builtin_amdgcn_global_load_lds((const __attribute__((address_space(1))) void*)(X + ((unsigned)(r * c_ldx) * 8u + coff)),
                                                     (__attribute__((address_space(3))) void*)dst, 16, 0, 0);
                }
            }
        }
        const unsigned a0p = fa + (unsigned)nbuf * (BM * BK * 8) + frag0;
        const unsigned x0p = fx + (unsigned)nbuf * (BN * BK * 8) + frag0;
#define VMX_G44_SECOND(i)                                                                                             \
        if constexpr (i < NI) {                                                                                           \
            _Pragma("unroll") for (int j = 0; j < FJ; ++j)                                                               \
                acc[i][j] = __builtin_amdgcn_mfma_f64_4x4x4f64(x1[i], a1[j], acc[i][j], 0, 0, 0);                        \
// ... 3 lines not shown
            __builtin_amdgcn_sched_barrier(0);                                                                           \
        }
        VMX_G44_SECOND(0) VMX_G44_SECOND(1) VMX_G44_SECOND(2) VMX_G44_SECOND(3)
        VMX_G44_SECOND(4) VMX_G44_SECOND(5) VMX_G44_SECOND(6) VMX_G44_SECOND(7)
#undef VMX_G44_SECOND
        lds_wait(a0, x0);
        buf = nbuf;
    }

    if (G.trace) t_loop = wall_clock64();
    if (pass + 1 < npass) {
        first_buf = (NBUF == 2 && epi_buf >= 0) ? epi_buf ^ 1 : 0;
        setup(pass + 1);
        if (!skip && kbeg < kend) dma_stage(kbeg, first_buf);
    }
    if (c_skip) continue;
    if constexpr (TAG == VMX_TAG_QUAD && NT == 256) {
        if (list && c_part) {
            const int c = lane & 15, r = lane >> 4;
            const bool first_seg = kbeg_c == 0;
#ifdef VMX_EPI_TRACE
            if (G.trace) t_first = wall_clock64();
#endif
            asm volatile("s_waitcnt vmcnt(0)" ::: "memory");
            __syncthreads();
#ifdef VMX_EPI_TRACE
            if (G.trace) t_e1 = wall_clock64();
#endif
            if (epi_buf < 0) {
#pragma unroll
                for (int i = 0; i < 8; ++i)
                    if (c == 0) c_part[((size_t)c_slot * 64 + wn + 4 * i + r) * 2 + (wave & 1)] = 0.0;
                continue;
            }
            const double* sE0 = &sA[epi_buf][0];
            const double* sE1 = &sX[epi_buf][0];
#pragma unroll
            for (int i = 0; i < 8; ++i) {
                const int n = c_n0 + wn + 4 * i + r;
                const int nc = n < c_N ? n : c_N - 1;
                const int e_n = wn + 4 * i + r;
                const double* e_row = (wn == 0 ? sE0 + e_n * BM : sE1 + (e_n - 32) * BM) + wm + c;
                const double* lin = c_lin;
                if (first_seg && c_lin_pool) {
                    const int mock = c_lin_row[nc];
                    lin += (size_t)(mock >= 0 ? 1 + mock : 0) * c_ldx;
                }
                double sum = 0.0;
#pragma unroll
                for (int jg = 0; jg < FJ / 4; ++jg) {
                    double tot[4];
#pragma unroll
                    for (int u = 0; u < 4; ++u) {
                        const double v = acc[i][4 * jg + u];
                        tot[u] = sum_k_quarters(v);
                    }
                    double out = fb == 0 ? tot[0] : fb == 1 ? tot[1] : fb == 2 ? tot[2] : tot[3];
                    const int m = c_m0 + wm + 16 * jg + c;
                    if (m < c_M) {
                        if (first_seg) out -= c_lin_pool ? lin[m] : sL[wm + 16 * jg + c];
                        sum = fma(e_row[16 * jg], 2.0 * out, sum);
                    }
                }
                sum = row_sum16(sum);
                if (c == 0) c_part[((size_t)c_slot * 64 + wn + 4 * i + r) * 2 + (wave & 1)] = n < c_N ? sum : 0.0;
            }
#ifdef VMX_EPI_TRACE
            if (G.trace) t_e2 = wall_clock64();
#endif
            continue;
        }
    }
#pragma unroll
    for (int i = 0; i < NI; ++i)
#pragma unroll
        for (int jg = 0; jg < FJ / 4; ++jg) {
            double tot[4];
#pragma unroll
            for (int u = 0; u < 4; ++u) {
                const double v = acc[i][4 * jg + u];
                tot[u] = sum_k_quarters(v);
            }
            const double out = fb == 0 ? tot[0] : fb == 1 ? tot[1] : fb == 2 ? tot[2] : tot[3];
            const int n = n0 + wn + 4 * i + (lane >> 4);
            const int m = c_m0 + wm + 16 * jg + (lane & 15);
            if (n < g.N && m < g.M) Dp[(size_t)n * g.ldd + m] = out;
        }
  }
    if (G.trace && threadIdx.x == 0 && !skip) {
        unsigned long long* tr = G.trace + 4 * ((size_t)blockIdx.y * gridDim.x + blockIdx.x);
#ifdef VMX_EPI_TRACE
        tr[0] = t_loop; tr[1] = t_first; tr[2] = t_e1; tr[3] = t_e2;
#else
        tr[0] = t_start; tr[1] = t_first; tr[2] = t_loop; tr[3] = wall_clock64();
#endif
    }
}

template <int NB>
__global__ __launch_bounds__(256) void k_csr_spmm(const int64_t* __restrict__ ptr, const int32_t* __restrict__ idx,
                                                  const double* __restrict__ val, int rows, const double* __restrict__ X,
                                                  int ldx, int N, double* __restrict__ Dp, int ldd)
{
    const int lane = threadIdx.x & 63;
    const int row = blockIdx.x * 4 + (threadIdx.x >> 6);
    if (row >= rows) return;
    const int n0 = blockIdx.y * NB;
    const int64_t k0 = ptr[row], k1 = ptr[row + 1];
    double acc[NB];
#pragma unroll
    for (int b = 0; b < NB; ++b) acc[b] = 0.0;
    int64_t k = k0 + lane;
    for (; k + 64 < k1; k += 128) {
        const int c0 = idx[k], c1 = idx[k + 64];
        const double v0 = val[k], v1 = val[k + 64];
#pragma unroll
        for (int b = 0; b < NB; ++b) {
            const double* x = X + (size_t)(n0 + b < N ? n0 + b : N - 1) * ldx;
            acc[b] = fma(v1, x[c1], fma(v0, x[c0], acc[b]));
        }
    }
    if (k < k1) {
        const int c0 = idx[k];
        const double v0 = val[k];
#pragma unroll
        for (int b = 0; b < NB; ++b) acc[b] = fma(v0, X[(size_t)(n0 + b < N ? n0 + b : N - 1) * ldx + c0], acc[b]);
    }
#pragma unroll
    for (int b = 0; b < NB; ++b) {
        double v = acc[b];
        for (int off = 32; off > 0; off >>= 1) v += __shfl_down(v, off, 64);
        if (lane == 0 && n0 + b < N) Dp[(size_t)(n0 + b) * ldd + row] = v;
    }
}

__global__ void k_quad_gather_csr(double* X, int ldx, const int64_t* ptr, const int32_t* idx, const double* val,
                                  const int32_t* mask_idx, int n_masked)
{
    const int i = blockIdx.x;
    if (i >= n_masked) return;
    const int r = mask_idx[i];
    for (int64_t k = ptr[r] + threadIdx.x; k < ptr[r + 1]; k += blockDim.x) X[(size_t)idx[k] * ldx + i] = val[k];
}

__global__ void k_sum_slabs(const double* __restrict__ part, double* __restrict__ y, int64_t count, int nslab)
{
    const int64_t i = (int64_t)blockIdx.x * blockDim.x + threadIdx.x;
    if (i >= count) return;
    double v = part[i];
    for (int s = 1; s < nslab; ++s) v += part[(int64_t)s * count + i];
    y[i] = v;
}

template <int NB>
__global__ __launch_bounds__(256) void k_gemv(GemmArgs g)
{
    const int batch = blockIdx.z;
    const double* A = g.A + batch * g.a_batch;
    const double* X = g.X + batch * g.x_batch;
    double* Dp = g.D + batch * g.d_batch;
    const int lane = threadIdx.x & 63;
    const int row = blockIdx.x * 4 + (threadIdx.x >> 6);
    if (row >= g.M) return;
    if (g.m_window && (row < g.m_window[0] || row > g.m_window[1])) return;
    const double* a = A + (size_t)row * g.lda;
    double acc[NB];
#pragma unroll
    for (int b = 0; b < NB; ++b) acc[b] = 0.0;
    const int K = g.tri ? min(g.K, (row + 2) & ~1) : g.K;
// ... 768 lines not shown
```

vega_amd/csrc/vmx_plan.h:

```cpp
#pragma once
#include <algorithm>
#include <cmath>
#include <cstdint>
#include <functional>
#include <string>
#include <vector>

struct GemmWork { int32_t prob, mt, nt, kbeg, kend, slab, slot, pad; };

namespace vmx_plan {

struct TapeProblem { int nq, nq_pad; };

inline int tape_row0(int nq, int bm) { const int r = nq % bm; return r % 2 == 0 ? r : 0; }
inline int tape_tile_hi(int nq, int mt, int bm)
{
    const int row0 = tape_row0(nq, bm);
    return row0 > 0 ? row0 + mt * bm : (mt + 1) * bm;
}
inline int tape_tile_stages(const TapeProblem& p, int mt, int bm, int bk) { return std::min((tape_tile_hi(p.nq, mt, bm) + bk - 1) / bk, p.nq_pad / bk); }

struct Tape {
    std::vector<GemmWork> work;
    std::vector<int32_t> queue;
    std::vector<int32_t> nt_off;
    std::vector<int32_t> piece_at;
    int n_blocks = 0, group_size = 1, n_pieces = 0;
    int64_t n_slots = 0;
    double capacity = 0.0;
};

inline Tape plan_quad_tape(const std::vector<TapeProblem>& probs, int tn, int blocks, double entry_stages, double skew,
                           int bm = 64, int bk = 32, bool k_bands = false)
{
    Tape T;
    const int P = std::max(blocks / 8 * 8, 8);
    struct Range { int prob, mt, stages; };
    std::vector<Range> ranges;
    for (size_t q = 0; q < probs.size(); ++q) {
        const int tm = (probs[q].nq + bm - 1) / bm;
        for (int mt = 0; mt < tm; ++mt) ranges.push_back({(int)q, mt, tape_tile_stages(probs[q], mt, bm, bk)});
    }
    std::stable_sort(ranges.begin(), ranges.end(), [](const Range& a, const Range& b) { return a.stages > b.stages; });
    const int gs = (tn % 4 == 0 && P / 8 >= 4) ? 4 : (tn % 2 == 0 && P / 8 >= 2) ? 2 : 1;
    const int n_groups = tn / gs, n_pieces = 8 * (P / 8 / gs);
    const double ovh = entry_stages;
    double stages_total = 0.0;
    for (auto& r : ranges) stages_total += (double)r.stages * n_groups;
    constexpr int MIN_SEG = 2;
    struct Entry { GemmWork w; int piece; };
    std::vector<Entry> entries;
    const int per_xcd_pieces = std::max(n_pieces / 8, 1);
    auto weight = [&](int pc) { return (pc % per_xcd_pieces) < per_xcd_pieces / 2 ? 1.0 + skew : 1.0 - skew; };
    auto fill = [&](double cap0, bool keep) {
        if (keep) entries.clear();
        int pc = 0;
        double cur = 0.0, cap = cap0 * weight(0);
        for (auto& r : ranges)
            for (int grp = 0; grp < n_groups; ++grp) {
                int k = 0, left = r.stages;
                while (left > 0) {
                    const double avail = cap - cur - ovh;
                    if (cur > 0.0 && avail < (double)std::min(left, MIN_SEG)) { ++pc; cur = 0.0; cap = cap0 * weight(std::min(pc, n_pieces - 1)); continue; }
                    int take = std::min(left, std::max(MIN_SEG, (int)std::floor(avail + 1e-9)));
                    const int rem = left - take;
                    if (rem > 0 && rem < MIN_SEG) take = (take - (MIN_SEG - rem) >= MIN_SEG) ? take - (MIN_SEG - rem) : left;
                    if (keep) entries.push_back({GemmWork{r.prob, r.mt, grp * gs, k * bk, (k + take) * bk, 0, 0, 0}, std::min(pc, n_pieces - 1)});
                    cur += take + ovh;
                    k += take; left -= take;
                }
            }
        return pc + 1;
    };
    {
        double lo = stages_total / n_pieces, hi = lo + ovh * (double)(ranges.size() * n_groups) / n_pieces + 4.0 * ovh + 256.0;
        if (per_xcd_pieces % 2) { lo /= 1.0 + std::fabs(skew); hi /= 1.0 - std::fabs(skew); }
        for (int it = 0; it < 48; ++it) {
            const double mid = 0.5 * (lo + hi);
            if (fill(mid, false) <= n_pieces) hi = mid; else lo = mid;
        }
        (void)fill(hi, true);
        T.capacity = hi;
    }
    std::vector<int32_t> nt_off(tn + 1, 0);
    for (auto& en : entries)
        for (int m = 0; m < gs; ++m) ++nt_off[en.w.nt + m + 1];
    for (int nt = 0; nt < tn; ++nt) nt_off[nt + 1] += nt_off[nt];
    {
        std::vector<int32_t> next(n_groups, 0);
        for (auto& en : entries) en.w.slot = next[en.w.nt / gs]++;
    }
    std::vector<int32_t> queue(P + 1, 0);
    std::vector<std::vector<GemmWork>> by_piece(n_pieces);
    for (auto& en : entries) by_piece[en.piece].push_back(en.w);
    std::vector<int32_t> piece_at(n_pieces);
    for (int pc = 0; pc < n_pieces; ++pc) piece_at[pc] = pc;
    if (k_bands && n_pieces >= 16) {
        std::vector<double> where(n_pieces, 0.0);
        for (int pc = 0; pc < n_pieces; ++pc) {
            double wsum = 0.0, ksum = 0.0;
            for (auto& w : by_piece[pc]) { const double len = w.kend - w.kbeg; wsum += len; ksum += len * 0.5 * (w.kbeg + w.kend); }
            where[pc] = wsum > 0.0 ? ksum / wsum : 1e300;
        }
        const int half = per_xcd_pieces / 2;
        std::vector<int32_t> heavy, light;
        for (int pc = 0; pc < n_pieces; ++pc) ((pc % per_xcd_pieces) < half ? heavy : light).push_back(pc);
        auto by_k = [&](int32_t a, int32_t b) { return where[a] < where[b]; };
        std::stable_sort(heavy.begin(), heavy.end(), by_k);
        std::stable_sort(light.begin(), light.end(), by_k);
        for (int x = 0; x < 8; ++x)
            for (int j = 0; j < per_xcd_pieces; ++j)
                piece_at[x * per_xcd_pieces + j] = j < half ? heavy[(size_t)x * half + j] : light[(size_t)x * (per_xcd_pieces - half) + (j - half)];
    }
    T.work.reserve(entries.size() * gs);
    for (int p = 0; p < P; ++p) {
        const int xcd = p % 8, i = p / 8, per_xcd = P / 8 / gs;
        const int member = i % gs;
        const int pos = xcd * per_xcd + i / gs;
        queue[p] = (int32_t)T.work.size();
        if (pos < n_pieces && i / gs < per_xcd)
            for (auto w : by_piece[piece_at[pos]]) {
                w.nt += member;
                w.slot += nt_off[w.nt];
                T.work.push_back(w);
            }
    }
    queue[P] = (int32_t)T.work.size();
    T.queue = std::move(queue);
    T.n_slots = nt_off[tn];
    T.nt_off = std::move(nt_off);
    T.n_blocks = P; T.group_size = gs; T.n_pieces = n_pieces;
    T.piece_at = std::move(piece_at);
    return T;
}

inline std::string check_quad_tape(const Tape& T, const std::vector<TapeProblem>& probs, int tn, double entry_stages, double skew,
                                   int bm = 64, int bk = 32)
{
    if ((int)T.queue.size() != T.n_blocks + 1 || (int)T.nt_off.size() != tn + 1) return "queue / nt_off sizes";
    if (T.queue[0] != 0 || T.queue[T.n_blocks] != (int32_t)T.work.size()) return "queue ends";
    for (int p = 0; p < T.n_blocks; ++p) if (T.queue[p + 1] < T.queue[p]) return "queue not monotone";
    std::vector<std::vector<std::vector<std::pair<int, int>>>> seg(probs.size());
    for (size_t q = 0; q < probs.size(); ++q) seg[q].resize((size_t)((probs[q].nq + bm - 1) / bm) * tn);
    std::vector<char> slot_used((size_t)T.n_slots, 0);
    for (auto& w : T.work) {
        if (w.prob < 0 || w.prob >= (int)probs.size()) return "problem index";
        const int tm = (probs[w.prob].nq + bm - 1) / bm;
        if (w.mt < 0 || w.mt >= tm || w.nt < 0 || w.nt >= tn) return "tile index";
        if (w.kbeg % bk || w.kend % bk || w.kend <= w.kbeg) return "segment not stage-aligned or empty";
        if (w.slot < T.nt_off[w.nt] || w.slot >= T.nt_off[w.nt + 1]) return "slot outside its walker tile's range";
        if (slot_used[w.slot]++) return "slot written twice";
        seg[w.prob][(size_t)w.mt * tn + w.nt].push_back({w.kbeg, w.kend});
    }
    for (auto u : slot_used) if (!u) return "slot never written";
    for (size_t q = 0; q < probs.size(); ++q) {
        const int tm = (probs[q].nq + bm - 1) / bm;
        for (int mt = 0; mt < tm; ++mt)
            for (int nt = 0; nt < tn; ++nt) {
                auto v = seg[q][(size_t)mt * tn + nt];
                std::sort(v.begin(), v.end());
                const int want = tape_tile_stages(probs[q], mt, bm, bk) * bk;
                int at = 0;
                for (auto& s : v) { if (s.first != at) return "K range has a gap or an overlap"; at = s.second; }
                if (at != want) return "K range not covered to its end";
            }
    }
    for (int nt = 0; nt < tn; ++nt) {
        std::vector<const GemmWork*> mine;
        for (auto& w : T.work) if (w.nt == nt) mine.push_back(&w);
        std::sort(mine.begin(), mine.end(), [](const GemmWork* a, const GemmWork* b) { return a->slot < b->slot; });
        for (size_t j = 1; j < mine.size(); ++j) {
            const GemmWork &a = *mine[j - 1], &b = *mine[j];
            if (a.prob == b.prob && a.mt == b.mt) { if (b.kbeg != a.kend) return "segments of a K range out of slot order"; continue; }
            const int la = tape_tile_stages(probs[a.prob], a.mt, bm, bk);
            const int lb = tape_tile_stages(probs[b.prob], b.mt, bm, bk);
            if (lb > la) return "row tiles out of tape order (long rows first)";
            if (b.kbeg != 0) return "a K range starts in the middle";
        }
    }
    const int gs = T.group_size, per_xcd = T.n_blocks / 8 / gs, per_xcd_pieces = std::max(T.n_pieces / 8, 1);
    for (int p = 0; p < T.n_blocks; ++p) {
        const int xcd = p % 8, i = p / 8, pos = xcd * per_xcd + i / gs;
        if (i / gs >= per_xcd) { if (T.queue[p + 1] != T.queue[p]) return "a surplus block has work"; continue; }
        const int pcs = T.piece_at[pos];
        if ((pcs % per_xcd_pieces < per_xcd_pieces / 2) != (pos % per_xcd_pieces < per_xcd_pieces / 2)) return "a piece sits on a position of the other weight class";
        double cost = 0.0;
        for (int j = T.queue[p]; j < T.queue[p + 1]; ++j) cost += (T.work[j].kend - T.work[j].kbeg) / bk + entry_stages;
        const double w = (pcs % per_xcd_pieces) < per_xcd_pieces / 2 ? 1.0 + skew : 1.0 - skew;
        if (cost > T.capacity * w + entry_stages + 4.0 + 1e-6) return "a piece exceeds its capacity by more than one entry";
        if (pcs + 1 < T.n_pieces && cost > 0.0 && cost < T.capacity * w - entry_stages - 4.0) {
            bool later = false;
            for (int p2 = 0; p2 < T.n_blocks && !later; ++p2) {
                if ((p2 / 8) / gs >= per_xcd) continue;
                const int pcs2 = T.piece_at[(p2 % 8) * per_xcd + (p2 / 8) / gs];
                if (pcs2 > pcs && T.queue[p2 + 1] > T.queue[p2]) later = true;
            }
            if (later) return "a piece before the last is short";
        }
        if (i % gs != 0) {
            const int lead = p - 8 * (i % gs);
            if (T.queue[p + 1] - T.queue[p] != T.queue[lead + 1] - T.queue[lead]) return "lock-step group members differ in length";
            for (int j = 0; j < T.queue[p + 1] - T.queue[p]; ++j) {
                const GemmWork &a = T.work[T.queue[lead] + j], &b = T.work[T.queue[p] + j];
                if (a.prob != b.prob || a.mt != b.mt || a.kbeg != b.kbeg || a.kend != b.kend || b.nt != a.nt + i % gs) return "lock-step group members differ";
            }
        }
    }
    return "";
}

struct SplitProblem { int tiles; int stages; int64_t slab_bytes; int max_split; int tm; int tn; };
inline std::vector<int> choose_group_splits(const std::vector<SplitProblem>& probs, bool two_per_cu = false)
{
    const int n = (int)probs.size();
    std::vector<int> best(n, 0);
    if (n == 0 || n > 3) return best;
    constexpr double BLOCK_OVERHEAD = 4.0;
    constexpr double STAGE_US = 0.85, SLAB_BYTES_PER_US = 3.0e6;
    double best_cost = 1e300;
    std::vector<int> cur(n, 1);
    const int combos = 1 << (2 * n);
    auto schedule = [](std::vector<double>& free_at, double cost, int blocks, double& makespan) {
        for (int b = 0; b < blocks; ++b) {
            std::pop_heap(free_at.begin(), free_at.end(), std::greater<double>());
            const double t = free_at.back() + cost;
            free_at.back() = t;
            std::push_heap(free_at.begin(), free_at.end(), std::greater<double>());
            if (t > makespan) makespan = t;
        }
    };
    for (int c = 0; c < combos; ++c) {
        bool ok = true;
        double penalty = 0.0;
        for (int i = 0; i < n; ++i) {
            cur[i] = 1 << ((c >> (2 * i)) & 3);
            if (cur[i] > probs[i].max_split || probs[i].stages / cur[i] < 4) ok = false;
            penalty += (cur[i] - 1) * 2.0 * (double)probs[i].slab_bytes / SLAB_BYTES_PER_US / STAGE_US;
        }
        if (!ok) continue;
        double makespan = 0.0;
        if (!two_per_cu) {
            std::vector<double> free_at(256, 0.0);
            for (int i = 0; i < n; ++i)
                schedule(free_at, (double)((probs[i].stages + cur[i] - 1) / cur[i]) + BLOCK_OVERHEAD, probs[i].tiles * cur[i], makespan);
        } else {
            for (int x = 0; x < 8; ++x) {
                std::vector<double> free_at(64, 0.0);
// ... 167 lines not shown
```

Baseline: 965,000.

## Evaluate quadratic chi2 via a triangular root factor of Q'

Adds a root form of the quadratic chi2. The inverse covariance is Cholesky-factored on the host, and the product with the marginalisation operator is reduced by Householder QR to a trapezoidal factor, so chi2 = ||R x||^2 - 2 lin·x + c0. The GEMM tape is reused with per-segment slab outputs instead of dot-product partials, and a new k_chi2_root kernel sums the segments, squares them and reduces. The cost model enables this path only when the trapezoid is cheaper than the triangular Q' GEMM, accepting extra setup (host sync, Cholesky, many QR launches) and more output traffic from slabs.

```diff
diff --git a/vega_amd/csrc/vegamx.hip b/vega_amd/csrc/vegamx.hip
--- a/vega_amd/csrc/vegamx.hip
+++ b/vega_amd/csrc/vegamx.hip
@@ -117,6 +117,7 @@
     DevBuf<double> marg, marg_out;
     DevBuf<double> q_mat, q_w, q_lin, q_c0, q_x0, q_x, q_z;
     DevBuf<double> q_u, q_f, q_u0, q_y;
+    DevBuf<double> q_root;
     DevBuf<double> mg_g, mg_c0, mg_y;
     DevBuf<double> mc_chol, mc_fid, q_cfull, q_m0, mc_z, mc_noise, mc_r0, mc_t;
     bool has_factor = false;
@@ -1632,6 +1633,8 @@
     DevBuf<int64_t> window;
 };
 
+constexpr bool QUAD_ROOT_DEFAULT = true;
+
 struct vmx_engine {
     int device = 0;
     hipStream_t stream = nullptr;
@@ -1726,7 +1729,10 @@
     int pad_l = 0, pad_r = 0;
     int fact_slab_rows = 0;
     std::map<int, std::vector<int>> group_splits;
-    struct QuadList { DevBuf<GemmWork> work; DevBuf<int32_t> queue, nt_off; DevBuf<double> part; int n_blocks = 0; int n_entries = 0; };
+    struct QuadList {
+        DevBuf<GemmWork> work; DevBuf<int32_t> queue, nt_off; DevBuf<double> part; int n_blocks = 0; int n_entries = 0;
+        bool root = false; DevBuf<double> ypart; DevBuf<int32_t> segs; std::vector<int64_t> y_off; std::vector<int32_t> seg_off; int max_segs = 0;
+    };
     std::map<int, QuadList*> quad_lists;
     std::vector<void*> host_allocs;
     std::map<int, QuadList*> cinv_lists;
@@ -1767,6 +1773,10 @@
     bool static_poly = true;
     int quad_kind = 0;
     bool quad_factored = false;
+    bool quad_root = false;
+    bool no_quad_root = false;
+    bool force_quad_root = false;
+    bool last_root = false;
     struct MargReq { double* out; int64_t ld_out; int32_t* status; };
     const MargReq* marg_req = nullptr;
     int marg_slab_rows = 0;
@@ -2809,6 +2819,8 @@
     }
     if (getenv("VMX_NO_TAB2")) e->no_tab2 = true;
     if (getenv("VMX_NO_CINV_TAPE")) e->no_cinv_tape = true;
+    if (getenv("VMX_NO_QUAD_ROOT") || (!QUAD_ROOT_DEFAULT && !getenv("VMX_QUAD_ROOT"))) e->no_quad_root = true;
+    if (getenv("VMX_QUAD_ROOT") && !std::strcmp(getenv("VMX_QUAD_ROOT"), "force")) e->force_quad_root = !e->no_quad_root;
     if (getenv("VMX_NO_PK_W")) e->no_pk_w = true;
     if (getenv("VMX_NO_HOST_REDUCE")) e->no_host_reduce = true;
     if (getenv("VMX_NO_XI_LEAN")) e->xi_lean = false;
@@ -3234,6 +3246,7 @@
 }
 
 constexpr double QUAD_ENTRY_STAGES = 4.0, QUAD_SKEW = 0.12;
+constexpr double QUAD_ROOT_ENTRY_STAGES = 2.5, QUAD_STAGE_US = 1.98, QUAD_ROOT_BYTES_PER_US = 3.0e6, QUAD_ROOT_REDUCER_STAGES = 2.0;
 constexpr bool QUAD_K_BANDS = true;
 
 static vmx_engine::QuadList* quad_build_tape(vmx_engine* e, int B)
@@ -3243,6 +3256,27 @@
     for (auto* it : e->items) probs.push_back({it->dev.nq, it->dev.nq_pad});
     vmx_plan::Tape T = vmx_plan::plan_quad_tape(probs, tn, e->quad_blocks, QUAD_ENTRY_STAGES, QUAD_SKEW, GEMM_BM, GEMM_BK, QUAD_K_BANDS);
     auto* ql = new vmx_engine::QuadList();
+    if (e->quad_root && !e->no_quad_root) {
+        std::vector<vmx_plan::TapeProblem> roots;
+        for (auto* it : e->items) roots.push_back({it->dev.n_masked, it->dev.nq_pad, it->dev.nq - it->dev.n_masked});
+        vmx_plan::Tape R = vmx_plan::plan_quad_tape(roots, tn, e->quad_blocks, QUAD_ROOT_ENTRY_STAGES, QUAD_SKEW, GEMM_BM, GEMM_BK, QUAD_K_BANDS, true);
+        double bytes = 0.0;
+        for (size_t q = 0; q < roots.size(); ++q)
+            for (int t = R.tile_off[q]; t < R.tile_off[q + 1]; ++t)
+                for (int nt = 0; nt < tn; ++nt) bytes += 8.0 * GEMM_BM * GEMM_BN * R.seg_count[(size_t)t * tn + nt];
+        const double reducer_stages = bytes / QUAD_ROOT_BYTES_PER_US / QUAD_STAGE_US + QUAD_ROOT_REDUCER_STAGES;
+        if ((R.capacity + reducer_stages < T.capacity || e->force_quad_root) && !R.work.empty()) {
+            ql->root = true;
+            ql->max_segs = R.max_segs;
+            int64_t y = 0;
+            for (size_t q = 0; q < roots.size(); ++q) {
+                ql->y_off.push_back(y); ql->seg_off.push_back(R.tile_off[q] * tn);
+                y += (int64_t)R.max_segs * tn * GEMM_BN * e->items[q]->dev.n_masked_pad;
+            }
+            if (ql->ypart.alloc((size_t)y, true) || ql->segs.upload(R.seg_count.data(), R.seg_count.size())) { delete ql; return nullptr; }
+            T = std::move(R);
+        }
+    }
     ql->n_blocks = T.n_blocks;
     ql->n_entries = (int)T.n_slots;
     if (T.work.empty()) T.work.push_back(GemmWork{-1, 0, 0, 0, 0, 0, 0, 0});
@@ -3265,6 +3299,12 @@
         g.tm = (d.nq + GEMM_BM - 1) / GEMM_BM; g.tn = (B + GEMM_BN - 1) / GEMM_BN;
         g.part = ql->part.p; g.lin = it->q_lin.p; g.lin_row = e->call_mock ? e->call_mock : e->mock_index.p; g.lin_pool = d.mock_pool ? 1 : 0;
         g.row0 = vmx_plan::tape_row0(d.nq, GEMM_BM);
+        if (ql->root) {
+            g.A = it->q_root.p; g.M = d.n_masked; g.tri = 0; g.part = nullptr;
+            g.D = ql->ypart.p + ql->y_off[q]; g.ldd = d.n_masked_pad; g.d_slab = (int64_t)g.tn * GEMM_BN * d.n_masked_pad;
+            g.tm = (d.n_masked + GEMM_BM - 1) / GEMM_BM;
+            g.row0 = vmx_plan::tape_row0(d.n_masked, GEMM_BM);
+        }
         G.p[G.n++] = g;
     }
     G.work = ql->work.p;
@@ -3904,12 +3944,29 @@
             return 0;
         }
         e->last_form = 1;
+        e->last_root = false;
         if (B > 8 && e->items.size() <= VMX_MAX_GROUP) {
             vmx_engine::QuadList* ql = quad_work_list(e, B);
             if (!ql) return -2;
             {
                 ScopedTimer t(e, KC_QUAD);
                 quad_launch_list(e, ql, B);
+            }
+            e->last_root = ql->root;
+            if (ql->root) {
+                RootArgs R{};
+                for (size_t q = 0; q < e->items.size(); ++q) {
+                    const ItemDev& d = e->items[q]->dev;
+                    const int tn = (B + GEMM_BN - 1) / GEMM_BN;
+                    R.p[q] = {ql->ypart.p + ql->y_off[q], (int64_t)tn * GEMM_BN * d.n_masked_pad, ql->segs.p + ql->seg_off[q],
+                              (int32_t)d.n_masked_pad, (int32_t)d.n_masked, vmx_plan::tape_row0(d.n_masked, GEMM_BM), tn};
+                }
+                ScopedTimer t(e, KC_CHI2);
+                hipLaunchKernelGGL(k_chi2_root, dim3(B), dim3(CHI2_ROOT_THREADS), 0, e->stream, D, B, R);
+                HIP_OK(hipGetLastError());
+                e->last_B = B;
+                e->last_full = false;
+                return 0;
             }
             ScopedTimer t(e, KC_CHI2);
 #ifdef VMX_EXP_SKIP_SMALL
@@ -4244,6 +4301,19 @@
         const bool fact = e->quad_kind == 2 || (e->quad_kind == 0 && cost_f < 0.75 * cost_q);
         if (fact != e->quad_factored) { e->quad_factored = fact; e->quad_mat_dirty = true; }
     }
+    bool want_root = !e->quad_factored && !e->no_quad_root && e->items.size() <= VMX_MAX_GROUP;
+    {
+        double tri = 0.0, trap = 0.0;
+        for (auto* it : e->items) {
+            int na = 0;
+            for (int q = 0; q < it->dev.n_bb[VMX_BB_POST_ADD]; ++q) na += it->dev.bb[VMX_BB_POST_ADD][q].n_coef;
+            const double nq = it->dev.d.n_model + na, nm = it->dev.n_masked;
+            if (nm > nq) want_root = false;
+            tri += 0.5 * nq * nq; trap += nm * nq - 0.5 * nm * nm;
+        }
+        if (!e->force_quad_root && !(trap < tri)) want_root = false;
+    }
+    bool root_ok = want_root, rebuilt = false;
     for (auto* it : e->items) {
         ItemDev& d = it->dev;
         const int nm = d.n_masked, nmp = d.n_masked_pad;
@@ -4343,6 +4413,39 @@
             if (it->q_mat.p == nullptr && it->q_mat.alloc((size_t)nq * nqp, true)) return -2;
             hipLaunchKernelGGL(k_half_from_full, dim3((nqp + 255) / 256, nq), dim3(256), 0, e->stream, it->q_mat.p, qfull.p, nq, nqp);
             if (marg_fold_matrix(e, it, X.p)) return -2;
+            rebuilt = true;
+            DevBuf<double> U, qr_part, qr_v, qr_row;
+            std::vector<double> hu;
+            if (root_ok) {
+                hu.assign((size_t)nm * nmp, 0.0);
+                if (it->has_cinv) {
+                    std::vector<double> hc((size_t)nm * nmp);
+                    HIP_OK(hipStreamSynchronize(e->stream));
+                    HIP_OK(hipMemcpy(hc.data(), cfull.p, hc.size() * sizeof(double), hipMemcpyDeviceToHost));
+                    if (!vmx_plan::cholesky_lower(hc.data(), nm, nmp)) {
+                        std::fprintf(stderr, "[vegamx] the inverse covariance of an item is not positive definite: chi2 keeps the Q' form\n");
+                        root_ok = false;
+                    }
+                    for (int i = 0; i < nm && root_ok; ++i)
+                        for (int m = 0; m <= i; ++m) hu[(size_t)m * nmp + i] = hc[(size_t)i * nmp + m];
+                } else
+                    for (int i = 0; i < nm; ++i) hu[(size_t)i * nmp + i] = 1.0;
+            }
+            if (root_ok) {
+                if (U.upload(hu.data(), hu.size())) return -2;
+                if (it->q_root.p == nullptr && it->q_root.alloc((size_t)nm * nqp, true)) return -2;
+                launch_product(e, KC_OTHER, X.p, nmp, 0, nq, nmp, U.p, nmp, 0, nm, it->q_root.p, nqp, 0, 1, nm);
+                const int chunks_max = (nm + QR_CH - 1) / QR_CH;
+                if (qr_part.alloc((size_t)chunks_max * nqp, true) || qr_v.alloc((size_t)nmp, true) || qr_row.alloc((size_t)nqp, true)) return -2;
+                for (int t = 0; t + 1 < nm; ++t) {
+                    const int r = nm - 1 - t, j = nq - 1 - t, chunks = r / QR_CH + 1;
+                    const dim3 grid((unsigned)(j / 256 + 1), (unsigned)chunks);
+                    hipLaunchKernelGGL(k_qr_dot, grid, dim3(256), 0, e->stream, (const double*)it->q_root.p, nqp, r, j, qr_part.p, qr_v.p, qr_row.p);
+                    hipLaunchKernelGGL(k_qr_apply, grid, dim3(256), 0, e->stream, it->q_root.p, nqp, r, j, chunks, (const double*)qr_part.p,
+                                       (const double*)qr_v.p, (const double*)qr_row.p);
+                }
+                HIP_OK(hipGetLastError());
+            }
             HIP_OK(hipStreamSynchronize(e->stream));
         }
         const int rows = 1 + it->n_mocks;
@@ -4384,6 +4487,14 @@
     std::vector<ItemDev> items;
     for (auto* it : e->items) items.push_back(it->dev);
     HIP_OK(hipMemcpy(e->d_items.p, items.data(), items.size() * sizeof(ItemDev), hipMemcpyHostToDevice));
+    if (rebuilt || e->quad_factored) {
+        const bool have = root_ok && !e->quad_factored;
+        if (have != e->quad_root) {
+            for (auto& q : e->quad_lists) delete q.second;
+            e->quad_lists.clear();
+        }
+        e->quad_root = have;
+    }
     e->quad_mat_dirty = false;
     e->quad_lin_dirty = false;
     e->last_B = 0;
@@ -6903,7 +7014,8 @@
         if (capacity >= 9) out[8] = e->last_form;
         if (capacity >= 10) out[9] = e->last_route | e->route_setup;
         if (capacity >= 11) out[10] = e->last_fft_form;
-        if (capacity >= 8) { out[7] = live[4]; return capacity >= 11 ? 11 : capacity >= 10 ? 10 : capacity >= 9 ? 9 : 8; }
+        if (capacity >= 12) out[11] = e->last_form == 1 && e->last_root ? 1 : 0;
+        if (capacity >= 8) { out[7] = live[4]; return capacity >= 12 ? 12 : capacity >= 11 ? 11 : capacity >= 10 ? 10 : capacity >= 9 ? 9 : 8; }
         return capacity >= 7 ? 7 : capacity >= 5 ? 5 : capacity >= 4 ? 4 : 3;
     }
     else if (what == 5) {
@@ -6989,6 +7101,12 @@
         src = e->odd_coef.p + P.odd_off; count = (int64_t)4 * P.odd_ncoef;
     }
     else if (what == 17) { src = e->metal_bias.p; count = (int64_t)B * 3 * (int64_t)e->metals.size(); if (count == 0) { fail(-1, "none: no metal terms"); return -1; } }
+    else if (what == 20 || what == 21) {
+        if (index < 0 || index >= (int)e->items.size()) { fail(-1, "invalid argument: item index"); return -1; }
+        const ItemHost* it = e->items[index];
+        if (e->quad_factored || !it->q_mat.p || (what == 20 && (!e->quad_root || !it->q_root.p))) { fail(-1, "none: the engine holds no such tensor of the Q' form"); return -1; }
+        src = what == 20 ? it->q_root.p : it->q_mat.p; count = (int64_t)(what == 20 ? it->dev.n_masked : it->dev.nq) * it->dev.nq_pad;
+    }
     else { fail(-1, "invalid argument: what"); return -1; }
     if (count > capacity) { fail(-1, "invalid argument: capacity too small"); return -1; }
     if (hipMemcpy(out, src, (size_t)count * sizeof(double), hipMemcpyDeviceToHost) != hipSuccess) { fail(-2, "hipMemcpy"); return -2; }
diff --git a/vega_amd/csrc/vmx_device.h b/vega_amd/csrc/vmx_device.h
--- a/vega_amd/csrc/vmx_device.h
+++ b/vega_amd/csrc/vmx_device.h
@@ -2051,6 +2051,122 @@
     }
 }
 
+struct RootItem { const double* y; int64_t slab; const int32_t* segs; int32_t ldy, rows, row0, tn; };
+struct RootArgs { RootItem p[VMX_MAX_GROUP]; };
+#define CHI2_ROOT_THREADS 1024
+
+__global__ __launch_bounds__(CHI2_ROOT_THREADS) void k_chi2_root(EngineDev D, int B, RootArgs R)
+{
+    constexpr int NWV = CHI2_ROOT_THREADS / 64;
+    const int b = blockIdx.x;
+    if (b >= B) return;
+    __shared__ double red[NWV];
+    const int nt = b >> 6, lane = threadIdx.x & 63;
+    const int wave = __builtin_amdgcn_readfirstlane(threadIdx.x >> 6);
+    const int mock = D.mock_index[b];
+    int st = D.status[b];
+    double tail = 0.0;
+    for (int q = 0; q < D.n_items; ++q) {
+        const ItemDev& it = D.items[q];
+        tail += it.q_c0[(mock >= 0 && it.mock_pool) ? 1 + mock : 0];
+    }
+    {
+        const double* t = D.theta + (size_t)b * D.n_params;
+        for (int q = 0; q < D.n_priors; ++q) {
+            const double dlt = t[D.prior_slot[q]] - D.prior_mean[q];
+            tail += dlt * dlt / (D.prior_sigma[q] * D.prior_sigma[q]);
+        }
+    }
+    double acc = 0.0;
+    for (int q = 0; q < D.n_items; ++q) {
+        const ItemDev& it = D.items[q];
+        const RootItem& r = R.p[q];
+        const double* y = r.y + (size_t)b * r.ldy + lane;
+        const int tm = (r.rows + 63) / 64;
+#pragma unroll 2
+        for (int mt = wave; mt < tm; mt += NWV) {
+            const int m0 = r.row0 > 0 ? (mt == 0 ? 0 : r.row0 + (mt - 1) * 64) : mt * 64;
+            const int mend = (r.row0 > 0 && mt == 0) ? r.row0 : min(m0 + 64, r.rows);
+            const int ns = r.segs[mt * r.tn + nt];
+            if (m0 + lane < mend) {
+                const double* ym = y + m0;
+                const double y0 = ym[0];
+                const double y1 = ns > 1 ? ym[r.slab] : 0.0;
+                const double y2 = ns > 2 ? ym[2 * r.slab] : 0.0;
+                const double y3 = ns > 3 ? ym[3 * r.slab] : 0.0;
+                double v = ((y0 + y1) + y2) + y3;
+                for (int s = 4; s < ns; ++s) v += ym[(size_t)s * r.slab];
+                acc = fma(v, v, acc);
+            }
+        }
+        const double* lin = it.q_lin + (size_t)((mock >= 0 && it.mock_pool) ? 1 + mock : 0) * it.nq_pad;
+        const double* x = it.q_x + (size_t)b * it.nq_pad;
+#pragma unroll 4
+        for (int j = threadIdx.x; j < it.nq; j += CHI2_ROOT_THREADS) acc = fma(-2.0 * lin[j], x[j], acc);
+    }
+    for (int off = 32; off > 0; off >>= 1) acc += __shfl_down(acc, off, 64);
+    if (lane == 0) red[wave] = acc;
+    __syncthreads();
+    if (threadIdx.x != 0) return;
+    double c = 0.0;
+    for (int w = 0; w < NWV; ++w) c += red[w];
+    c += tail;
+    if (!(c == c) || c > 1e300 || c < -1e300) { st |= VMX_STATUS_NONFINITE; D.status[b] = st; }
+    D.chi2[b] = st ? 1e100 : c;
+    if (D.chi2_host) D.chi2_host[b] = st ? 1e100 : c;
+    if (D.status_host) D.status_host[b] = st;
+    if (b == 0) {
+        D.k_live[2] = D.coef_win[0]; D.k_live[3] = D.coef_win[1]; D.coef_win[0] = 0x7fffffff; D.coef_win[1] = -1;
+        xtab_key_store(D);
+    }
+}
+
+#define QR_CH 128
+__global__ __launch_bounds__(256) void k_qr_dot(const double* F, int ld, int r, int j, double* part, double* v, double* rowr)
+{
+    __shared__ double sx[QR_CH];
+    const int c = blockIdx.x * 256 + threadIdx.x;
+    const int i0 = blockIdx.y * QR_CH, i1 = min(i0 + QR_CH, r + 1);
+    if (threadIdx.x < i1 - i0) {
+        const double x = F[(size_t)(i0 + threadIdx.x) * ld + j];
+        sx[threadIdx.x] = x;
+        if (blockIdx.x == 0) v[i0 + threadIdx.x] = x;
+    }
+    __syncthreads();
+    if (c > j) return;
+    if (blockIdx.y == 0) rowr[c] = F[(size_t)r * ld + c];
+    const double* col = F + (size_t)i0 * ld + c;
+    double s = 0.0;
+#pragma unroll 8
+    for (int i = 0; i < i1 - i0; ++i) s = fma(sx[i], col[(size_t)i * ld], s);
+    part[(size_t)blockIdx.y * ld + c] = s;
+}
+
+__global__ __launch_bounds__(256) void k_qr_apply(double* F, int ld, int r, int j, int chunks, const double* part, const double* v,
+                                                  const double* rowr)
+{
+    const int c = blockIdx.x * 256 + threadIdx.x;
+    const int i0 = blockIdx.y * QR_CH, i1 = min(i0 + QR_CH, r + 1);
+    if (c > j) return;
+    double sigma = 0.0, d = 0.0;
+    for (int ch = 0; ch < chunks; ++ch) { sigma += part[(size_t)ch * ld + j]; d += part[(size_t)ch * ld + c]; }
+    if (!(sigma > 0.0)) return;
+    const double xr = v[r];
+    const double alpha = xr >= 0.0 ? -sqrt(sigma) : sqrt(sigma);
+    const double tau = 1.0 / (sigma - alpha * xr);
+    const double w = -tau * (d - alpha * rowr[c]);
+    double* col = F + (size_t)i0 * ld + c;
+    if (c == j) {
+        for (int i = i0; i < i1; ++i) col[(size_t)(i - i0) * ld] = i == r ? alpha : 0.0;
+        return;
+    }
+#pragma unroll 4
+    for (int i = i0; i < i1; ++i) {
+        const double vi = i == r ? xr - alpha : v[i];
+        col[(size_t)(i - i0) * ld] = fma(w, vi, col[(size_t)(i - i0) * ld]);
+    }
+}
+
 struct MargOutItem { const double* y; const double* c0; int32_t item, n, ld, off, slabs, pad; };
 struct MargOutArgs { MargOutItem p[VMX_MAX_MARG]; double* out; int64_t ld_out; int32_t* status_out; int32_t finish; };
 
@@ -2443,6 +2559,8 @@
     int p_M = g.M, p_N = g.N, p_lda = g.lda, p_ldx = g.ldx, p_lin_pool = g.lin_pool, p_row0 = g.row0;
     int p_mend = g.M;
     double* p_part = g.part;
+    double* p_D = Dp;
+    int p_ldd = g.ldd;
     const double* p_lin = g.lin;
     const int32_t* p_lin_row = g.lin_row;
 
@@ -2468,6 +2586,7 @@
             A = (const char*)q.A; X = (const char*)q.X;
             p_M = q.M; p_N = q.N; p_lda = q.lda; p_ldx = q.ldx; p_lin_pool = q.lin_pool; p_row0 = q.row0;
             p_part = q.part; p_lin = q.lin; p_lin_row = q.lin_row;
+            p_D = q.D + (int64_t)__builtin_amdgcn_readfirstlane(wk.slab) * q.d_slab; p_ldd = q.ldd;
             n0 = wk.nt * BN;
             slot = wk.slot;
         }
@@ -2517,6 +2636,8 @@
     const int c_m0 = m0, kbeg_c = kbeg, kend_c = kend, c_n0 = n0, c_slot = slot, c_first = first_buf;
     const int c_M = p_mend, c_N = p_N, c_ldx = p_ldx, c_lin_pool = p_lin_pool;
     double* const c_part = p_part;
+    double* const c_D = p_D;
+    const int c_ldd = p_ldd;
     const double* const c_lin = p_lin;
     const int32_t* const c_lin_row = p_lin_row;
     const bool c_skip = skip;
@@ -2686,9 +2807,9 @@
                 tot[u] = sum_k_quarters(v);
             }
             const double out = fb == 0 ? tot[0] : fb == 1 ? tot[1] : fb == 2 ? tot[2] : tot[3];
-            const int n = n0 + wn + 4 * i + (lane >> 4);
+            const int n = c_n0 + wn + 4 * i + (lane >> 4);
             const int m = c_m0 + wm + 16 * jg + (lane & 15);
-            if (n < g.N && m < g.M) Dp[(size_t)n * g.ldd + m] = out;
+            if (n < c_N && m < c_M) c_D[(size_t)n * c_ldd + m] = out;
         }
   }
     if (G.trace && threadIdx.x == 0 && !skip) {
diff --git a/vega_amd/csrc/vmx_plan.h b/vega_amd/csrc/vmx_plan.h
--- a/vega_amd/csrc/vmx_plan.h
+++ b/vega_amd/csrc/vmx_plan.h
@@ -10,7 +10,7 @@
 
 namespace vmx_plan {
 
-struct TapeProblem { int nq, nq_pad; };
+struct TapeProblem { int nq, nq_pad; int k_off = 0; };
 
 inline int tape_row0(int nq, int bm) { const int r = nq % bm; return r % 2 == 0 ? r : 0; }
 inline int tape_tile_hi(int nq, int mt, int bm)
@@ -18,7 +18,7 @@
     const int row0 = tape_row0(nq, bm);
     return row0 > 0 ? row0 + mt * bm : (mt + 1) * bm;
 }
-inline int tape_tile_stages(const TapeProblem& p, int mt, int bm, int bk) { return std::min((tape_tile_hi(p.nq, mt, bm) + bk - 1) / bk, p.nq_pad / bk); }
+inline int tape_tile_stages(const TapeProblem& p, int mt, int bm, int bk) { return std::min((p.k_off + tape_tile_hi(p.nq, mt, bm) + bk - 1) / bk, p.nq_pad / bk); }
 
 struct Tape {
     std::vector<GemmWork> work;
@@ -28,10 +28,12 @@
     int n_blocks = 0, group_size = 1, n_pieces = 0;
     int64_t n_slots = 0;
     double capacity = 0.0;
+    std::vector<int32_t> seg_count, tile_off;
+    int max_segs = 0;
 };
 
 inline Tape plan_quad_tape(const std::vector<TapeProblem>& probs, int tn, int blocks, double entry_stages, double skew,
-                           int bm = 64, int bk = 32, bool k_bands = false)
+                           int bm = 64, int bk = 32, bool k_bands = false, bool segments = false)
 {
     Tape T;
     const int P = std::max(blocks / 8 * 8, 8);
@@ -58,14 +60,15 @@
         double cur = 0.0, cap = cap0 * weight(0);
         for (auto& r : ranges)
             for (int grp = 0; grp < n_groups; ++grp) {
-                int k = 0, left = r.stages;
+                int k = 0, left = r.stages, seg = 0;
                 while (left > 0) {
                     const double avail = cap - cur - ovh;
                     if (cur > 0.0 && avail < (double)std::min(left, MIN_SEG)) { ++pc; cur = 0.0; cap = cap0 * weight(std::min(pc, n_pieces - 1)); continue; }
                     int take = std::min(left, std::max(MIN_SEG, (int)std::floor(avail + 1e-9)));
                     const int rem = left - take;
                     if (rem > 0 && rem < MIN_SEG) take = (take - (MIN_SEG - rem) >= MIN_SEG) ? take - (MIN_SEG - rem) : left;
-                    if (keep) entries.push_back({GemmWork{r.prob, r.mt, grp * gs, k * bk, (k + take) * bk, 0, 0, 0}, std::min(pc, n_pieces - 1)});
+                    if (keep) entries.push_back({GemmWork{r.prob, r.mt, grp * gs, k * bk, (k + take) * bk, segments ? seg : 0, 0, 0}, std::min(pc, n_pieces - 1)});
+                    ++seg;
                     cur += take + ovh;
                     k += take; left -= take;
                 }
@@ -112,6 +115,17 @@
             for (int j = 0; j < per_xcd_pieces; ++j)
                 piece_at[x * per_xcd_pieces + j] = j < half ? heavy[(size_t)x * half + j] : light[(size_t)x * (per_xcd_pieces - half) + (j - half)];
     }
+    if (segments) {
+        T.tile_off.assign(probs.size() + 1, 0);
+        for (size_t q = 0; q < probs.size(); ++q) T.tile_off[q + 1] = T.tile_off[q] + (probs[q].nq + bm - 1) / bm;
+        T.seg_count.assign((size_t)T.tile_off[probs.size()] * tn, 0);
+        for (auto& en : entries)
+            for (int m = 0; m < gs; ++m) {
+                int32_t& n = T.seg_count[(size_t)(T.tile_off[en.w.prob] + en.w.mt) * tn + en.w.nt + m];
+                n = std::max(n, en.w.slab + 1);
+                T.max_segs = std::max(T.max_segs, (int)n);
+            }
+    }
     T.work.reserve(entries.size() * gs);
     for (int p = 0; p < P; ++p) {
         const int xcd = p % 8, i = p / 8, per_xcd = P / 8 / gs;
@@ -140,8 +154,14 @@
     if ((int)T.queue.size() != T.n_blocks + 1 || (int)T.nt_off.size() != tn + 1) return "queue / nt_off sizes";
     if (T.queue[0] != 0 || T.queue[T.n_blocks] != (int32_t)T.work.size()) return "queue ends";
     for (int p = 0; p < T.n_blocks; ++p) if (T.queue[p + 1] < T.queue[p]) return "queue not monotone";
-    std::vector<std::vector<std::vector<std::pair<int, int>>>> seg(probs.size());
-    for (size_t q = 0; q < probs.size(); ++q) seg[q].resize((size_t)((probs[q].nq + bm - 1) / bm) * tn);
+    std::vector<std::vector<std::vector<std::pair<int, int>>>> seg(probs.size()), seg_slab(probs.size());
+    for (size_t q = 0; q < probs.size(); ++q) { seg[q].resize((size_t)((probs[q].nq + bm - 1) / bm) * tn); seg_slab[q].resize(seg[q].size()); }
+    const bool segments = !T.seg_count.empty();
+    if (segments) {
+        if (T.tile_off.size() != probs.size() + 1 || T.tile_off[0] != 0) return "tile_off size";
+        for (size_t q = 0; q < probs.size(); ++q) if (T.tile_off[q + 1] - T.tile_off[q] != (probs[q].nq + bm - 1) / bm) return "tile_off steps";
+        if (T.seg_count.size() != (size_t)T.tile_off[probs.size()] * tn) return "seg_count size";
+    }
     std::vector<char> slot_used((size_t)T.n_slots, 0);
     for (auto& w : T.work) {
         if (w.prob < 0 || w.prob >= (int)probs.size()) return "problem index";
@@ -151,6 +171,8 @@
         if (w.slot < T.nt_off[w.nt] || w.slot >= T.nt_off[w.nt + 1]) return "slot outside its walker tile's range";
         if (slot_used[w.slot]++) return "slot written twice";
         seg[w.prob][(size_t)w.mt * tn + w.nt].push_back({w.kbeg, w.kend});
+        seg_slab[w.prob][(size_t)w.mt * tn + w.nt].push_back({w.kbeg, w.slab});
+        if (!segments && w.slab != 0) return "a slab index on a tape without segments";
     }
     for (auto u : slot_used) if (!u) return "slot never written";
     for (size_t q = 0; q < probs.size(); ++q) {
@@ -163,6 +185,13 @@
                 int at = 0;
                 for (auto& s : v) { if (s.first != at) return "K range has a gap or an overlap"; at = s.second; }
                 if (at != want) return "K range not covered to its end";
+                if (segments) {
+                    auto u = seg_slab[q][(size_t)mt * tn + nt];
+                    std::sort(u.begin(), u.end());
+                    for (size_t j = 0; j < u.size(); ++j) if (u[j].second != (int)j) return "segment indices of a K range not dense in K order";
+                    if (T.seg_count[(size_t)(T.tile_off[q] + mt) * tn + nt] != (int32_t)u.size()) return "seg_count differs from the range's entries";
+                    if ((int)u.size() > T.max_segs) return "a range has more segments than max_segs";
+                }
             }
     }
     for (int nt = 0; nt < tn; ++nt) {
```

After: 1.013 million (median of 6 runs). +5.0%, better.
